# tatsuya-ogawa/GaussianSplattingMlx

Hardware: AMD Instinct MI355X
Metric: train views/sec (full step: fwd + L1/DSSIM loss + bwd + Adam + densify/prune at the reference cadence), Lego 800x800 300k Gaussians (higher is better)
Workload: dtype f32; 1 GPU; c3_300k_800: synthetic Lego cameras 800x800, N=300000 trained-like Gaussians, SH degree 4 (K=25), 16x16 tiles, 100 views, 1 view per rank per step, mode train; mode=train, parallelism=dp1, rccl_ranks=1, view_assignment=rank r renders view (step * world + r) mod views; parameters replicated, views_per_rank=1, N=300000, W=800, H=800, tile=16

## Files before the change

gaussiansplattingmlx_amd/_lib.py:

```python
from __future__ import annotations

import ctypes as C
import os

HERE = os.path.dirname(os.path.abspath(__file__))
LIB_PATH = os.environ.get("GSPLAT_LIB", os.path.join(HERE, "libgsplat_hip.so"))

GS_OK = 0
MAX_FEATURE_CHANNELS = 256
STATUS = {1: "GS_ERR_INVALID_ARG", 2: "GS_ERR_SIZE_MISMATCH", 3: "GS_ERR_WORKSPACE_OVERFLOW", 4: "GS_ERR_HIP",
          5: "GS_ERR_NO_FORWARD", 6: "GS_ERR_NO_DEVICE", 7: "GS_ERR_IO", 8: "GS_ERR_COMM", 9: "GS_ERR_REPLICA_MISMATCH"}
GS_ERR_REPLICA_MISMATCH = 9


class GsplatError(RuntimeError):
    def __init__(self, code, msg):
        super().__init__(f"{STATUS.get(code, code)}: {msg}")
        self.code = code


class gs_camera(C.Structure):
    _fields_ = [("view", C.c_float * 16), ("proj", C.c_float * 16), ("cam_center", C.c_float * 3),
                ("fov_x", C.c_float), ("fov_y", C.c_float), ("focal_x", C.c_float), ("focal_y", C.c_float)]

# ... 99 lines not shown
    "gs_ssim_forward": (C.c_int, [_vp] + [C.c_int] * 4 + [_vp] * 9),
    "gs_ssim_backward": (C.c_int, [_vp] + [C.c_int] * 4 + [_vp] * 11),
    "gs_render_forward": (C.c_int, [_vp, C.c_int, C.c_int] + [_vp] * 6 + [C.POINTER(gs_camera)] + [_vp] * 4),
    "gs_render_backward": (C.c_int, [_vp] + [_vp] * 9),
    "gs_render_backward_dp": (C.c_int, [_vp] + [_vp] * 8),
    "gs_render_backward_adam": (C.c_int, [_vp] * 7 + [C.c_longlong, _vp, C.c_float, C.c_float, C.c_float, C.c_float]),
    "gs_render_backward_dp_begin": (C.c_int, [_vp] * 5),
    "gs_render_backward_dp_finish": (C.c_int, [_vp] * 5),
    "gs_render_backward_dp_finish_geom": (C.c_int, [_vp] * 6),
    "gs_render_backward_dp_geom": (C.c_int, [_vp] * 10),
    "gs_sh_grad_from_views_adam_dir": (C.c_int, [_vp, C.c_int, C.c_int, C.c_int] + [_vp] * 9 + [C.c_longlong] + [C.c_float] * 6 + [_vp]),
    "gs_adam_step_add": (C.c_int, [_vp, C.c_longlong] + [_vp] * 4 + [C.c_int, _vp, _vp] + [C.c_float] * 4 + [_vp, C.c_longlong]),
    "gs_sh_grad_from_views": (C.c_int, [_vp, C.c_int, C.c_int, C.c_int] + [_vp] * 5),
    "gs_accum_grad_norm": (C.c_int, [_vp, C.c_int, _vp, _vp, _vp]),
    "gs_classify_gaussians": (C.c_int, [_vp, C.c_int, _vp, C.c_float, _vp, C.c_int, _vp, C.c_float, C.c_float,
                                        C.c_float, C.c_int, _vp, _vp]),
    "gs_densify_offsets": (C.c_int, [_vp, C.c_int, _vp, _vp, _vp, _vp]),
    "gs_build_densify_output_map": (C.c_int, [_vp, C.c_int, _vp, _vp, C.c_int, _vp, _vp]),
    "gs_densify_gather": (C.c_int, [_vp, C.c_int, C.c_int] + [_vp] * 15),
    "gs_densify_plan": (C.c_int, [_vp, C.c_int, _vp, _vp, _vp]),
    "gs_densify_plan_read": (C.c_int, [_vp, C.c_int, _vp, C.POINTER(C.c_int)]),
    "gs_build_densify_output_map_planned": (C.c_int, [_vp, C.c_int, _vp, _vp, C.c_int, _vp, _vp]),
    "gs_densify_gather_planned": (C.c_int, [_vp, C.c_int, C.c_int] + [_vp] * 8 + [C.c_ulonglong] + [_vp] * 6),
    "gs_densify_gather_planned_packed": (C.c_int, [_vp, C.c_int, C.c_int] + [_vp] * 8 + [C.c_ulonglong, _vp, C.POINTER(C.c_int)]),
    "gs_densify_noise": (C.c_int, [_vp, C.c_ulonglong, C.c_int, _vp]),
    "gs_ply_write": (C.c_int, [_vp, C.c_char_p, C.c_int, C.c_int] + [_vp] * 6),
    "gs_ply_probe": (C.c_int, [_vp, C.c_char_p, _vp, _vp, _vp]),
    "gs_ply_load": (C.c_int, [_vp, C.c_char_p, C.c_int, C.c_int] + [_vp] * 6),
    "gs_ply_pack_rows": (C.c_int, [_vp, C.c_int, C.c_int] + [_vp] * 7),
    "gs_set_block_work_buffer": (C.c_int, [_vp, _vp]),
    "gs_view_hint_words": (C.c_int, [_vp, C.POINTER(C.c_int)]),
    "gs_set_view_hints": (C.c_int, [_vp, _vp, C.c_int]),
    "gs_set_depth_cuts": (C.c_int, [_vp, C.c_int]),
    "gs_clear_depth_cuts": (C.c_int, [_vp, _vp, C.c_int]),
    "gs_forward_missed": (C.c_int, [_vp, C.POINTER(C.c_int)]),
    "gs_cut_stats": (C.c_int, [_vp, C.POINTER(C.c_uint32)]),
    "gs_set_grad_norm_accum": (C.c_int, [_vp, _vp]),
    "gs_block_count": (C.c_int, [_vp, _vp]),
    "gs_copy_block_work": (C.c_int, [_vp, _vp]),
    "gs_dist_topk": (C.c_int, [_vp, C.c_int, C.c_int, C.c_int, C.c_int, _vp, _vp]),
    "gs_sh_grad_from_views_adam": (C.c_int, [_vp, C.c_int, C.c_int, C.c_int] + [_vp] * 8 + [C.c_longlong] + [C.c_float] * 6),
    "gs_loss_target_cache_floats": (C.c_int, [_vp, C.POINTER(C.c_longlong)]),
    "gs_set_loss_target_cache": (C.c_int, [_vp, _vp, C.c_int]),
    "gs_set_loss_mask": (C.c_int, [_vp, _vp]),
    "gs_loss_forward_backward": (C.c_int, [_vp] + [_vp] * 5 + [C.c_float, C.c_float] + [_vp] * 3),
    "gs_depth_loss": (C.c_int, [_vp, C.POINTER(gs_depth_loss_params)] + [_vp] * 7),
    "gs_depth_normalize": (C.c_int, [_vp, C.c_longlong, _vp, _vp, C.c_float, _vp]),
    "gs_normal_loss": (C.c_int, [_vp, C.POINTER(gs_normal_loss_params)] + [_vp] * 9),
    "gs_depth_normals": (C.c_int, [_vp, C.POINTER(C.c_float), C.c_int, C.c_int, _vp, _vp, C.c_float, C.c_float, _vp]),
    "gs_image_metrics": (C.c_int, [_vp, C.c_int, C.c_int] + [_vp] * 4),
    "gs_colour_moments": (C.c_int, [_vp, C.c_longlong] + [_vp] * 4),
    "gs_adam_step": (C.c_int, [_vp, C.c_longlong] + [_vp] * 4 + [C.c_int, _vp, _vp] + [C.c_float] * 4),
    "gs_profile_enable": (C.c_int, [_vp, C.c_uint]),
    "gs_profile_read": (C.c_int, [_vp, _vp, _vp]),
    "gs_copy_last_contrib": (C.c_int, [_vp, _vp]),
    "gs_last_stats": (C.c_int, [_vp, C.POINTER(C.c_uint32)]),
    "gs_ctx_set_tuning": (C.c_int, [_vp, C.c_int, C.c_longlong]),
    "gs_copy_overflow_flag": (C.c_int, [_vp, _vp]),
    "gs_set_update_gate": (C.c_int, [_vp, _vp]),
    "gs_set_overflow_rider": (C.c_int, [_vp, _vp]),
    "gs_set_pose_correction": (C.c_int, [_vp, _vp, _vp]),
    "gs_set_exposure": (C.c_int, [_vp, _vp, _vp]),
    "gs_apply_exposure": (C.c_int, [_vp, C.c_longlong, _vp, _vp, _vp]),
    "gs_set_bilateral_grid": (C.c_int, [_vp, _vp, _vp, C.c_int, C.c_int, C.c_int, C.c_float]),
    "gs_apply_bilateral_grid": (C.c_int, [_vp, C.c_int, C.c_int, _vp, C.c_int, C.c_int, C.c_int, _vp, _vp]),
    "gs_set_antialiasing": (C.c_int, [_vp, C.c_int]),
    "gs_set_camera_model": (C.c_int, [_vp, C.c_int]),
    "gs_get_camera_model": (C.c_int, [_vp, C.POINTER(C.c_int)]),
    "gs_set_sh_degree": (C.c_int, [_vp, C.c_int]),
    "gs_get_sh_degree": (C.c_int, [_vp, C.POINTER(C.c_int)]),
    "gs_set_background": (C.c_int, [_vp, _vp]),
    "gs_get_background": (C.c_int, [_vp, _vp]),
    "gs_composite_target": (C.c_int, [_vp, C.c_longlong, _vp, _vp, _vp, _vp]),
    "gs_set_absgrad": (C.c_int, [_vp, C.c_int]),
    "gs_get_absgrad": (C.c_int, [_vp, C.c_int, _vp]),
    "gs_set_adc_stats": (C.c_int, [_vp, _vp, _vp, _vp]),
    "gs_adc_accumulate": (C.c_int, [_vp, C.c_int, _vp, _vp, C.c_int, _vp, _vp, _vp]),
    "gs_adc_classify": (C.c_int, [_vp, C.c_int] + [_vp] * 4 + [C.c_int, _vp, C.POINTER(gs_adc_params), C.c_int, C.c_int, _vp, _vp]),
    "gs_adc_gather": (C.c_int, [_vp, C.c_int, C.c_int] + [_vp] * 9 + [C.c_int] + [_vp] * 6),
    "gs_adc_gather_moments": (C.c_int, [_vp, C.c_int, C.c_int, _vp, _vp, _vp, C.POINTER(_vp), C.POINTER(_vp)]),
    "gs_adc_reset_opacity": (C.c_int, [_vp, C.c_int, _vp, _vp, _vp, C.c_float]),
    "gs_set_sparse_adam": (C.c_int, [_vp, C.c_int]),
    "gs_get_visibility": (C.c_int, [_vp, C.c_int, _vp]),
    "gs_adam_step_visible": (C.c_int, [_vp, C.c_longlong] + [_vp] * 4 + [C.c_int, _vp, _vp, _vp] + [C.c_float] * 4 + [C.c_int, _vp]),
    "gs_set_filter3d_cameras": (C.c_int, [_vp, C.c_int, _vp]),
    "gs_compute_filter3d": (C.c_int, [_vp, C.c_int, _vp, _vp]),
    "gs_set_filter3d": (C.c_int, [_vp, _vp]),
    "gs_filter3d_bake": (C.c_int, [_vp, C.c_int] + [_vp] * 5),
    "gs_undistort": (C.c_int, [_vp, C.POINTER(gs_lens)] + [C.c_int] * 6 + [_vp, _vp, _vp]),
    "gs_undistort_fisheye": (C.c_int, [_vp, C.POINTER(gs_fisheye_lens)] + [C.c_int] * 6 + [_vp, _vp, _vp]),
    "gs_tsdf_integrate": (C.c_int, [_vp, C.POINTER(gs_tsdf_grid), C.c_int, C.POINTER(gs_tsdf_view)] + [_vp] * 4),
    "gs_tsdf_mesh_workspace_bytes": (C.c_size_t, [C.POINTER(gs_tsdf_grid)]),
    "gs_tsdf_mesh_plan": (C.c_int, [_vp, C.POINTER(gs_tsdf_grid), _vp, _vp, C.c_float, _vp, C.c_size_t, C.POINTER(C.c_longlong)]),
    "gs_tsdf_mesh_emit": (C.c_int, [_vp, C.POINTER(gs_tsdf_grid), _vp, _vp, _vp, _vp, C.c_float, _vp, _vp, _vp, _vp]),
    "gs_set_mcmc": (C.c_int, [_vp, _vp]),
    "gs_mcmc_regularizer_grad": (C.c_int, [_vp, C.c_int] + [_vp] * 5),
    "gs_mcmc_inject_noise": (C.c_int, [_vp, C.c_int] + [_vp] * 4 + [C.c_float, _vp]),
    "gs_mcmc_random": (C.c_int, [_vp, C.c_ulonglong, C.c_int, C.c_int, C.c_int, _vp, _vp, _vp]),
    "gs_mcmc_relocate": (C.c_int, [_vp, C.c_int, C.c_int] + [_vp] * 11),
    "gs_mcmc_grow": (C.c_int, [_vp, C.c_int, C.c_int, C.c_int] + [_vp] * 11),
    "gs_set_gathered_gate": (C.c_int, [_vp, C.c_longlong, C.c_int, _vp]),
    "gs_set_gate_seen": (C.c_int, [_vp, _vp]),
    "gs_dp_cc_floats": (C.c_longlong, [C.c_int]),
    "gs_dp_check_replicas": (C.c_int, [_vp, C.c_int, _vp, C.c_longlong]),
    "gs_dp_check_replicas_begin": (C.c_int, [_vp, C.c_int, _vp, C.c_longlong]),
    "gs_dp_check_replicas_end": (C.c_int, [_vp]),
    "gs_dp_check_plan": (C.c_int, [_vp, C.POINTER(C.c_longlong), C.c_int]),
}

_lib = None


def load():
    global _lib
    if _lib is not None:
        return _lib
    if not os.path.exists(LIB_PATH):
        raise ImportError(f"{LIB_PATH} is missing: run `python -m gaussiansplattingmlx_amd.build` "
                          "(or __graft_entry__.build()). There is no CPU fallback.")
    import torch
    lib = C.CDLL(LIB_PATH)
    for name, (res, args) in _SIGS.items():
        fn = getattr(lib, name)
        fn.restype = res
        fn.argtypes = args
    _lib = lib
    return lib


TUNE_FWD_WAVES_PER_SIMD, TUNE_BWD_WAVES_PER_CU, TUNE_FWD_QUADRANTS, TUNE_OP_FWD_PPL, TUNE_OP_BWD_PPL, \
    TUNE_FWD_TRACE_BUFFER, TUNE_DEPTH_GRADIENT, TUNE_WIDE_TILE_SORT, TUNE_HOST_OVERFLOW_ERRORS, TUNE_SPLITTER_DEPTH_SORT, \
    TUNE_COLOUR_RIDERS, TUNE_FWD_QUEUES, TUNE_FWD_FOUR_WAVES, TUNE_FWD_FOLD_TEST_SCALE, TUNE_POISON_CHECKPOINTS, TUNE_RENDER_ONLY, TUNE_FWD_PAIR, TUNE_FWD_SLOW_SLOT, TUNE_TRIM_RECTS, TUNE_SH_BAND_SKIP = range(20)


def exported_symbols():
    return list(_SIGS)


def make_camera(view, proj, camCenter, fovX, fovY, focalX, focalY) -> gs_camera:
    import numpy as np
    cam = gs_camera()
    v = np.asarray(view, dtype=np.float32).reshape(16)
    p = np.asarray(proj, dtype=np.float32).reshape(16)
    cc = np.asarray(camCenter, dtype=np.float32).reshape(3)
    for i in range(16):
        cam.view[i] = float(v[i])
        cam.proj[i] = float(p[i])
    for i in range(3):
        cam.cam_center[i] = float(cc[i])
    cam.fov_x, cam.fov_y, cam.focal_x, cam.focal_y = float(fovX), float(fovY), float(focalX), float(focalY)
    return cam
```

gaussiansplattingmlx_amd/build.py:

```python
from __future__ import annotations

import os
import subprocess
import sys
from concurrent.futures import ThreadPoolExecutor

HERE = os.path.dirname(os.path.abspath(__file__))
CSRC = os.path.join(HERE, "csrc")
LIB = os.path.join(HERE, "libgsplat_hip.so")
HIPCC = os.environ.get("HIPCC", "/opt/rocm/bin/hipcc")
ARCH = "gfx950"

SOURCES = {
    "api.hip": [],
    "projection.hip": ["-ffp-contract=off"],
    "binning.hip": ["-ffp-contract=off"],
    "blend.hip": [],
    "blend_v2.hip": ["-ffp-contract=off"],
    "ssim.hip": [],
    "optim.hip": [],
    "densify.hip": ["-ffp-contract=off"],
    "adc.hip": ["-ffp-contract=off"],
    "ply.hip": [],
    "knn.hip": ["-ffp-contract=off"],
    "dp.hip": [],
    "mcmc.hip": ["-ffp-contract=off"],
    "exposure.hip": ["-ffp-contract=off"],
    "bilateral_grid.hip": ["-ffp-contract=off"],
    "filter3d.hip": ["-ffp-contract=off"],
    "contrib.hip": ["-ffp-contract=off"],
    "features.hip": ["-ffp-contract=off"],
    "background.hip": ["-ffp-contract=off"],
    "depth_loss.hip": ["-ffp-contract=off"],
    "normal_loss.hip": ["-ffp-contract=off"],
    "lens.hip": ["-ffp-contract=off"],
    "metrics.hip": ["-ffp-contract=off"],
    "tsdf.hip": ["-ffp-contract=off"],
}
COMMON = ["-O3", "-std=c++17", "-fPIC", f"--offload-arch={ARCH}", "-fvisibility=hidden", "-Wall", "-fno-slp-vectorize",
          "-Wno-unused-function", "-DGSPLAT_BUILD"]


def _newer(target, deps):
    if not os.path.exists(target):
        return False
    t = os.path.getmtime(target)
    return all(os.path.getmtime(d) <= t for d in deps)


def build(force: bool = False, verbose: bool = False, variant: str = "", defines=()) -> str:
    headers = [os.path.join(CSRC, h) for h in os.listdir(CSRC) if h.endswith(".h")]
    headers.append(os.path.join(HERE, "..", "include", "gsplat.h"))
    objdir = os.path.join(HERE, "_obj" + ("_" + variant if variant else ""))
    lib = LIB if not variant else os.path.join(HERE, f"libgsplat_hip_{variant}.so")
    os.makedirs(objdir, exist_ok=True)
    jobs = []
    objs = []
    for src, extra in SOURCES.items():
        s = os.path.join(CSRC, src)
        o = os.path.join(objdir, src.replace(".hip", ".o"))
        objs.append(o)
        if force or not _newer(o, [s] + headers + [os.path.abspath(__file__)]):
            jobs.append([HIPCC, *COMMON, *extra, *defines, "-c", s, "-o", o])

    def run(cmd):
        if verbose:
            print(" ".join(cmd), flush=True)
        r = subprocess.run(cmd, capture_output=True, text=True)
        if r.returncode != 0:
            raise RuntimeError("hipcc failed:\n" + " ".join(cmd) + "\n" + r.stdout + r.stderr)
        if verbose and r.stderr.strip():
            print(r.stderr)

    if jobs:
        with ThreadPoolExecutor(max_workers=min(4, len(jobs))) as ex:
            list(ex.map(run, jobs))
    if jobs or not os.path.exists(lib):
        run([HIPCC, "-shared", "-fPIC", f"--offload-arch={ARCH}", "-o", lib, *objs, "-ldl"])
    return lib


if __name__ == "__main__":
    argv = sys.argv[1:]
    variant = argv[argv.index("--variant") + 1] if "--variant" in argv else ""
    print(build(force="--force" in argv, verbose=True, variant=variant, defines=[a for a in argv if a.startswith("-D")]))
```

gaussiansplattingmlx_amd/csrc/api.hip:

```cpp
#include <math.h>
#include <stdlib.h>
#include <stdio.h>
#include <string.h>

#include "gs_ctx.h"
#include <vector>

using namespace gs;

namespace {

int fail(gs_ctx* c, int code, const std::string& msg)
{
    if (c) c->err = msg;
    return code;
}

void free_gaussian_ws(gs_ctx* c)
{
    ctx_free(c, c->packed12); ctx_free(c, c->gradAcc16);
    for (int i = 0; i < 2; i++) { ctx_free(c, c->depthKey[i]); ctx_free(c, c->depthVal[i]); }
    ctx_free(c, c->tilesTouched); ctx_free(c, c->tileRect); ctx_free(c, c->tilePieces); ctx_free(c, c->waveSeg);
    ctx_free(c, c->scanPrefix); ctx_free(c, c->scanTmp); ctx_free(c, c->blockSums);
    ctx_free(c, c->visPerBlock); ctx_free(c, c->dropPerBlock);
// ... 385 lines not shown
    c->blocksX = gs_div_up(W, 16); c->blocksY = gs_div_up(H, 16);
    c->real.tileW = tile_w; c->real.tileH = tile_h; c->real.gridW = c->gridW; c->real.gridH = c->gridH; c->real.T = c->T;
    c->real.fast16 = c->fast16;
    {
        const char* e = getenv("GSPLAT_BLOCK_LISTS");
        const int nbx = gs_div_up(tile_w, 16), nby = gs_div_up(tile_h, 16);
        if (!c->fast16 && !(e && atoi(e) == 0) && (long long)c->gridW * nbx <= 65535 && (long long)c->gridH * nby <= 65535) {
            c->virt.nbx = nbx; c->virt.nby = nby; c->virt.tw = tile_w; c->virt.th = tile_h;
            c->tileW = 16; c->tileH = 16;
            c->gridW *= nbx; c->gridH *= nby;
            c->T = c->gridW * c->gridH;
            c->fast16 = true;
            c->blocksX = c->gridW; c->blocksY = c->gridH;
        }
    }
    if (const char* e = getenv("GSPLAT_COLOUR_RIDERS")) c->colourRiders = atoi(e);
    if (const char* e = getenv("GSPLAT_FWD_WIDE")) c->fwdWide = atoi(e) < 0 ? -1 : atoi(e) != 0;
    if (const char* e = getenv("GSPLAT_FWD_QUEUES")) { const int q = atoi(e); if (q >= 1 && q <= (int)GS_QUEUES && !(q & (q - 1))) c->fwdQueues = q; }
    if (const char* e = getenv("GSPLAT_RIDER_SHARES")) {
        int vals[GS_RIDE_HOSTS + 1], n = 0;
        for (const char* q = e; *q && n <= GS_RIDE_HOSTS; n++) {
            vals[n] = atoi(q);
            while (*q && *q != ',') q++;
            if (*q == ',') q++;
        }
        if (n == GS_RIDE_HOSTS) for (int i = 0; i < GS_RIDE_HOSTS; i++) c->riderShare[i] = vals[i];
        else fprintf(stderr, "gsplat: GSPLAT_RIDER_SHARES needs %d comma-separated values (got %s): ignored\n", GS_RIDE_HOSTS, e);
    }
    if (c->gridW > 65535 || c->gridH > 65535) { delete c; return GS_ERR_INVALID_ARG; }
    int bits = 1;
    while ((1LL << bits) < c->T) bits++;
    c->tileBits = bits;
    for (bits = 1; (1LL << bits) < c->real.T; bits++) {}
    c->real.tileBits = bits;
    auto bail = [&](int code) { gs_ctx_destroy(c); return code; };
    if (hipSetDevice(device) != hipSuccess) return bail(GS_ERR_HIP);
    if (hipStreamCreateWithFlags(&c->own_stream, hipStreamNonBlocking) != hipSuccess) return bail(GS_ERR_HIP);
    c->stream = c->own_stream;
    const size_t P = (size_t)W * H;
    c->numPixBlocks = c->blocksX * c->blocksY;
    c->opBlocks = c->real.fast16 ? c->numPixBlocks : c->real.T * gs_div_up(tile_w, 16) * gs_div_up(tile_h, 16);
    const size_t maxBlocks = (size_t)(c->opBlocks > c->numPixBlocks ? c->opBlocks : c->numPixBlocks);
    if (ctx_alloc(c, &c->blockWorkOwn, maxBlocks) || ctx_alloc(c, &c->blockOrder, maxBlocks + 8) || ctx_alloc(c, &c->fwdQueue, GS_QUEUES * GS_QUEUE_STRIDE) || ctx_alloc(c, &c->bwdQueue, GS_QUEUES * GS_QUEUE_STRIDE) ||
        ctx_alloc(c, &c->segBase, (size_t)c->numPixBlocks) || ctx_alloc(c, &c->finalT, P))
        return bail(GS_ERR_HIP);
    c->blockWork = c->blockWorkOwn;
    {
        hipDeviceProp_t prop;
        if (hipGetDeviceProperties(&prop, device) == hipSuccess && prop.multiProcessorCount > 0)
            c->numCUs = prop.multiProcessorCount;
    }
    if (ctx_alloc(c, &c->superCut, (size_t)c->T + 16) || ctx_alloc(c, &c->tileRanges, (size_t)c->T * 2) || ctx_alloc(c, &c->tileCounts, (size_t)c->T) ||
        ctx_alloc(c, &c->lastContrib, P) ||
        ctx_alloc(c, &c->lossPartials, (size_t)(c->lossPartialBlocks = gs_div_up(W, 16) * gs_div_up(H, 16) * 3) * 4 + 16) || ctx_alloc(c, &c->windowDev, 121) ||
        ctx_alloc(c, &c->counters, GS_CNT_COUNT) || ctx_alloc(c, &c->rowTotal, 256) ||
        ctx_alloc(c, &c->sortBits, GS_SMALL_SORT_BLOCKS) || ctx_alloc(c, &c->wideTotal, GS_WIDE_BINS) ||
        ctx_alloc(c, &c->bucketStart, 520) || ctx_alloc(c, &c->sortSplit[0], 256) || ctx_alloc(c, &c->sortSplit[1], 256))
        return bail(GS_ERR_HIP);
    if (ctx_alloc_pinned(c, &c->countersHost, GS_CNT_COUNT)) return bail(GS_ERR_HIP);
    if (ctx_alloc_pinned(c, &c->missHost, 16, hipHostMallocMapped)) return bail(GS_ERR_HIP);
    for (int i = 0; i < 16; i++) c->missHost[i] = 0;
    if (hipHostGetDevicePointer((void**)&c->missDev, c->missHost, 0) != hipSuccess) return bail(GS_ERR_HIP);
    if (hipEventCreateWithFlags(&c->fwdDone, hipEventDisableTiming) != hipSuccess) return bail(GS_ERR_HIP);
    float win[121];
    gs_ssim_window(11, 1.5f, win);
    if (hipMemcpy(c->windowDev, win, sizeof win, hipMemcpyHostToDevice) != hipSuccess) return bail(GS_ERR_HIP);
    if (hipMemset(c->counters, 0, sizeof(uint32_t) * GS_CNT_COUNT) != hipSuccess) return bail(GS_ERR_HIP);
    if (hipMemset(c->tileRanges, 0, sizeof(uint32_t) * 2 * c->T) != hipSuccess) return bail(GS_ERR_HIP);
    c->adamGate = c->counters + GS_CNT_OVERFLOW;
    *out = c;
    return GS_OK;
}

int gs_ctx_destroy(gs_ctx* c)
{
    if (!c) return GS_OK;
    (void)hipSetDevice(c->device);
    if (c->stream) (void)hipStreamSynchronize(c->stream);
    (void)gs_dp_shutdown(c);
    c->mem.freeAll();
    for (auto& e : c->profPool) { (void)hipEventDestroy(e.a); (void)hipEventDestroy(e.b); }
    if (c->fwdDone) (void)hipEventDestroy(c->fwdDone);
    if (c->densifyDone) (void)hipEventDestroy(c->densifyDone);
    if (c->own_stream) (void)hipStreamDestroy(c->own_stream);
    delete c;
    return GS_OK;
}

int gs_ctx_set_stream(gs_ctx* c, void* hip_stream)
{
    if (!c) return GS_ERR_INVALID_ARG;
    GS_HIP_CHECK(c, hipStreamSynchronize(c->stream));
    c->stream = (hipStream_t)hip_stream;
    return GS_OK;
}

int gs_ctx_reserve(gs_ctx* c, int max_gaussians, long long max_pairs)
{
    if (!c || max_gaussians < 0 || max_pairs < 0) return fail(c, GS_ERR_INVALID_ARG, "gs_ctx_reserve: negative size");
    (void)hipSetDevice(c->device);
    GS_HIP_CHECK(c, hipStreamSynchronize(c->stream));
    if (c->missHost[4] == 2u || c->arenaRegrowPending) {
        uint32_t parts[8], used = 0;
        GS_HIP_CHECK(c, hipMemcpy(parts, c->counters + GS_CNT_QSLOTS, sizeof parts, hipMemcpyDeviceToHost));
        for (uint32_t x : parts) used += x;
        const long long need5 = (((long long)used + c->fwd.qslotStatic) * c->fwd.statePlanes + 4) / 5;
        c->qslotWanted = need5 + need5 / 2 + 4096;
        const long long half = c->qslotCap + c->qslotCap / 2;
        if (c->qslotWanted < half) c->qslotWanted = half;
    }
    c->reserving = max_pairs > 0;
    int rc = ensure_capacity(c, max_gaussians, max_pairs);
    if (rc == GS_OK) rc = ensure_arena(c);
    c->reserving = false;
    if (rc == GS_OK) {
        if (max_pairs > 0) c->pairsReserved = true;
        c->missHost[4] = 0; c->arenaRegrowPending = false;
    }
    return rc;
}

size_t gs_workspace_bytes(const gs_ctx* c) { return c ? c->mem.deviceBytes : 0; }

int gs_sync(gs_ctx* c)
{
    if (!c) return GS_ERR_INVALID_ARG;
    const int rc = read_counters(c);
    if (rc) return rc;
    if (c->missHost[4]) {
        const uint32_t need = c->missHost[5];
        const int orc = overflow_error(c, need);
        if (c->missHost[4] == 2u) { c->arenaRegrowPending = true; c->fwd.arenaOverflow = true; }
        c->missHost[4] = 0;
        return orc;
    }
    if (c->countersHost[GS_CNT_OVERFLOW]) return overflow_error(c);
    return GS_OK;
}

int gs_overflow_pending(gs_ctx* c, uint32_t out[2])
{
    if (!c || !out) return GS_ERR_INVALID_ARG;
    out[0] = c->missHost ? c->missHost[4] : 0u;
    out[1] = c->missHost ? c->missHost[5] : 0u;
    if (out[0] == 0u && c->arenaRegrowPending) out[0] = 2u;
    return GS_OK;
}

int gs_wait(gs_ctx* c)
{
    if (!c) return GS_ERR_INVALID_ARG;
    GS_HIP_CHECK(c, hipStreamSynchronize(c->stream));
    return GS_OK;
}

const char* gs_last_error(const gs_ctx* c) { return c ? c->err.c_str() : "null context"; }

int gs_projection_forward(gs_ctx* c, int N, int K, const float* scales, const float* rotations, const float* means3d,
                          const float* shs, const gs_camera* cam, float* means2d, float* depths, float* color,
                          float* cov2d, float* conic, float* radii, float* rect_min, float* rect_max)
{
    if (!c) return GS_ERR_INVALID_ARG;
    if (N < 0 || K < 1 || !cam) return fail(c, GS_ERR_INVALID_ARG, "gs_projection_forward: bad N/K/cam");
    if ((c->modes.degree + 1) * (c->modes.degree + 1) > K) return fail(c, GS_ERR_SIZE_MISMATCH, "K smaller than (degree+1)^2");
    if (N > 0 && (!scales || !rotations || !means3d || !shs || !means2d || !depths || !color || !cov2d || !conic ||
                  !radii || !rect_min || !rect_max))
// ... 188 lines not shown

int gs_blend_features(gs_ctx* c, int N, int C, const float* packed, const float* features, float* out)
{
    if (!c) return GS_ERR_INVALID_ARG;
    if (const int prc = blend_features_preflight(c, "gs_blend_features", N, C, packed, features, out)) return prc;
    RealGeomScope real(c);
    c->fwd.valid = false; c->fwd.bwdPrepared = false;
    if (const int rc = launch_pack11_to_12(c, N, packed)) return rc;
    return launch_blend_features(c, C, features, out);
}

int gs_blend_features_backward(gs_ctx* c, int N, int C, const float* packed, const float* cot, float* grad_features)
{
    if (!c) return GS_ERR_INVALID_ARG;
    if (const int prc = blend_features_preflight(c, "gs_blend_features_backward", N, C, packed, cot, grad_features)) return prc;
    RealGeomScope real(c);
    c->fwd.valid = false; c->fwd.bwdPrepared = false;
    if (const int rc = launch_pack11_to_12(c, N, packed)) return rc;
    return launch_blend_features_backward(c, C, cot, grad_features);
}

int gs_feature_channel_group(void) { return feature_channel_group(); }

int gs_ssim_window(int K, float sigma, float* window)
{
    if (K <= 0 || K > 32 || !window) return GS_ERR_INVALID_ARG;
    float g[32];
    const float center = (float)K / 2.0f;
    float sum = 0.0f;
    for (int x = 0; x < K; x++) {
        const float d = (float)x - center;
        g[x] = expf(-(d * d) / (2.0f * (sigma * sigma)));
        sum += g[x];
    }
    for (int x = 0; x < K; x++) g[x] = g[x] / sum;
    for (int i = 0; i < K; i++)
        for (int j = 0; j < K; j++) window[i * K + j] = g[i] * g[j];
    return GS_OK;
}

int gs_ssim_forward(gs_ctx* c, int H, int W, int C, int K, const float* img1, const float* img2, const float* window,
                    float* out_ssim, float* out_mu1, float* out_mu2, float* out_sigma1, float* out_sigma2,
                    float* out_sigma12)
{
    if (!c) return GS_ERR_INVALID_ARG;
    if (H < 0 || W < 0 || C < 0 || K <= 0 || K > 32) return fail(c, GS_ERR_INVALID_ARG, "gs_ssim_forward: bad shape");
    if (C > 65535) return fail(c, GS_ERR_INVALID_ARG, "gs_ssim_forward: too many channels");
    if ((size_t)H * W * C > 0 && (!img1 || !img2 || !window || !out_ssim || !out_mu1 || !out_mu2 || !out_sigma1 ||
                                  !out_sigma2 || !out_sigma12))
        return fail(c, GS_ERR_INVALID_ARG, "gs_ssim_forward: null buffer");
    return launch_ssim_forward(c, H, W, C, K, img1, img2, window, out_ssim, out_mu1, out_mu2, out_sigma1, out_sigma2,
                               out_sigma12);
}

int gs_ssim_backward(gs_ctx* c, int H, int W, int C, int K, const float* grad_out, const float* img1,
                     const float* img2, const float* window, const float* mu1, const float* mu2, const float* sigma1,
                     const float* sigma2, const float* sigma12, float* grad_img1, float* grad_img2)
{
    if (!c) return GS_ERR_INVALID_ARG;
    if (H < 0 || W < 0 || C < 0 || K <= 0 || K > 32) return fail(c, GS_ERR_INVALID_ARG, "gs_ssim_backward: bad shape");
    if ((size_t)H * W * C > 0 && (!grad_out || !img1 || !img2 || !window || !mu1 || !mu2 || !sigma1 || !sigma2 ||
                                  !sigma12 || !grad_img1 || !grad_img2))
        return fail(c, GS_ERR_INVALID_ARG, "gs_ssim_backward: null buffer");
    return launch_ssim_backward(c, H, W, C, K, grad_out, 0.0f, img1, img2, window, mu1, mu2, sigma1, sigma2, sigma12,
                                grad_img1, grad_img2, 0.0f);
}

int gs_render_forward(gs_ctx* c, int N, int K, const float* xyz, const float* features_dc,
                      const float* features_rest, const float* scales, const float* rotation, const float* opacity,
                      const gs_camera* cam, float* out_color, float* out_depth, float* out_alpha, float* radii)
{
    if (!c) return GS_ERR_INVALID_ARG;
    if (N < 0 || K < 1 || !cam) return fail(c, GS_ERR_INVALID_ARG, "gs_render_forward: bad N/K/cam");
    if ((c->modes.degree + 1) * (c->modes.degree + 1) > K) return fail(c, GS_ERR_SIZE_MISMATCH, "K smaller than (degree+1)^2");
    if (!out_color || !out_alpha) return fail(c, GS_ERR_INVALID_ARG, "gs_render_forward: null output");
    if (N > 0 && (!xyz || !features_dc || (K > 1 && !features_rest) || !scales || !rotation || !opacity))
        return fail(c, GS_ERR_INVALID_ARG, "gs_render_forward: null parameter tensor");
    if (c->modes.fisheye && c->modes.poseDelta)
        return fail(c, GS_ERR_INVALID_ARG, "gs_render_forward: the fisheye camera model has no pose refinement (gs_set_pose_correction is set)");
    if (c->modes.fisheye && c->modes.filter3d)
        return fail(c, GS_ERR_INVALID_ARG, "gs_render_forward: the fisheye camera model has no 3-D filter (gs_set_filter3d is set)");
    c->fwd.valid = false;
    c->visN = -1;
    const bool keepRadii = c->sparseAdam || c->adcGradSum != nullptr;
    if (keepRadii && N > c->visCap) {
        if (const int arc = ctx_grow_pair(c, &c->visMask, &c->visRadii, &c->visCap, N > c->capN ? N : c->capN)) return arc;
    }
    if (keepRadii && !radii) radii = c->visRadii;
    c->binIsBlockLists = c->virt.nbx != 0;
    const bool reserved = c->pairsReserved && c->capN >= N;
    if (reserved) { const int orc = deferred_overflow(c); if (orc) return orc; }
    if (c->fwd.cutsActive && !c->fwd.missChecked) GS_HIP_CHECK(c, hipEventSynchronize(c->fwdDone));
    c->fwd.missed = false;
    c->fwd.bwdPrepared = false;
    c->fwd.arenaOverflow = false;
    c->fwd.cutStore = c->cutStore;
    c->fwd.cutsActive = c->cutStore != nullptr && c->allowCuts && N > 0;
    c->fwd.missChecked = !c->fwd.cutsActive;
    if (c->fwd.cutsActive) c->missHost[0] = 0;
    const CamParams cp = make_cam(cam, c->W, c->H);
    if (c->modes.poseDelta) {
        if (const int arc = ctx_grow(c, &c->posePartials, &c->posePartialsCap, pose_partials_floats(N))) return arc;
        if (const int prc = launch_pose_camera(c, cp, c->modes.poseDelta)) return prc;
    }
    c->segBaseWanted = c->fast16 && N > 0;
    c->segBaseDone = false;
    c->fwdPairNow = c->fast16 && blend_forward_v2_pair_decide(c);
    int rc = bin_with_capacity(c, N, reserved, !c->fast16, [&]() {
        return launch_projection_fused_forward(c, N, K, xyz, features_dc, features_rest, scales, rotation, opacity, cp,
                                               radii);
    });
    c->segBaseWanted = false;
    if (rc) { c->rider.on = false; return rc; }
    if (c->rider.on && c->rider.next < c->rider.total) {
        GsStageTimer t(c, GS_STAGE_PROJ_FWD, true);
        if ((rc = launch_colour_rest(c))) return rc;
    }
    c->rider.on = false;
    {
        GsStageTimer t(c, GS_STAGE_BLEND_FWD);
        rc = c->fast16 ? launch_blend_forward_v2(c, out_color, out_depth, out_alpha)
                       : launch_blend_forward(c, c->modes.bg, out_color, out_depth, out_alpha, c->lastContrib);
        if (rc) return rc;
    }
    if (c->fwd.cutsActive) GS_HIP_CHECK(c, hipEventRecord(c->fwdDone, c->stream));
    c->fwd.valid = true;
    c->absgradN = -1;
    c->fwd.blendBackwardDone = false;
    c->fwd.consumed = false;
    c->fwd.blockWork = c->blockWork;
    c->fwd.N = N; c->fwd.K = K;
    c->fwd.xyz = xyz; c->fwd.fdc = features_dc; c->fwd.frest = features_rest; c->fwd.scales = scales;
    c->fwd.rot = rotation; c->fwd.opacity = opacity;
    c->fwd.outColor = out_color; c->fwd.outDepth = out_depth; c->fwd.outAlpha = out_alpha;
    c->fwd.cam = cp;
    c->fwd.modes = c->modes;
    c->fwd.radii = keepRadii ? radii : nullptr;
    if (c->sparseAdam) c->visN = N;
    return GS_OK;
}

int gs_set_sparse_adam(gs_ctx* c, int enable)
{
    if (!c) return GS_ERR_INVALID_ARG;
    if (enable != 0 && enable != 1) return fail(c, GS_ERR_INVALID_ARG, "gs_set_sparse_adam: enable is 0 or 1");
    if (enable && c->mcmcOn)
        return fail(c, GS_ERR_INVALID_ARG, "gs_set_sparse_adam: the MCMC strategy is set (its noise and regularisers act on every Gaussian)");
    if (enable && c->modes.filter3d) return fail(c, GS_ERR_INVALID_ARG, "gs_set_sparse_adam: a 3-D filter is set (gs_set_filter3d)");
    c->sparseAdam = enable == 1;
    return GS_OK;
}

int gs_get_visibility(gs_ctx* c, int N, unsigned char* out)
{
    if (!c) return GS_ERR_INVALID_ARG;
    if (c->visN < 0)
        return fail(c, GS_ERR_NO_FORWARD, "gs_get_visibility: the last gs_render_forward was not made with sparse Adam on (gs_set_sparse_adam)");
    if (N != c->visN) return fail(c, GS_ERR_SIZE_MISMATCH, "gs_get_visibility: N differs from the forward's N");
    if (N > 0 && !out) return fail(c, GS_ERR_INVALID_ARG, "gs_get_visibility: null buffer");
    if (N > 0) GS_HIP_CHECK(c, hipMemcpyAsync(out, c->visMask, (size_t)N, hipMemcpyDeviceToDevice, c->stream));
    return GS_OK;
}

int gs_set_absgrad(gs_ctx* c, int enable)
{
    if (!c) return GS_ERR_INVALID_ARG;
// ... 435 lines not shown
    c->bgGrad = grad;
    c->bgW = grid_w;
    c->bgH = grid_h;
    c->bgL = grid_l;
    c->bgTv = tv_weight;
    return GS_OK;
}

int gs_apply_bilateral_grid(gs_ctx* c, int W, int H, const float* grid, int grid_w, int grid_h, int grid_l, const float* in,
                            float* out)
{
    if (!c) return GS_ERR_INVALID_ARG;
    if (W < 0 || H < 0) return fail(c, GS_ERR_INVALID_ARG, "gs_apply_bilateral_grid: negative image size");
    if (!bilateral_shape_ok(grid_w, grid_h, grid_l))
        return fail(c, GS_ERR_INVALID_ARG, "gs_apply_bilateral_grid: grid_w, grid_h in [2, 64] and grid_l in [2, 32]");
    if ((long long)W * H > 0 && (!grid || !in || !out)) return fail(c, GS_ERR_INVALID_ARG, "gs_apply_bilateral_grid: null buffer");
    return launch_bilateral_apply(c, W, H, grid, grid_w, grid_h, grid_l, in, out);
}

int gs_render_backward(gs_ctx* c, const float* cot_color, const float* cot_depth, const float* cot_alpha,
                       float* grad_xyz, float* grad_features_dc, float* grad_features_rest, float* grad_scales,
                       float* grad_rotation, float* grad_opacity)
{
    if (!c) return GS_ERR_INVALID_ARG;
    { const int prc = backward_preflight(c, "gs_render_backward", cot_depth != nullptr); if (prc) return prc; }
    const int N = c->fwd.N, K = c->fwd.K;
    if (!cot_color) return fail(c, GS_ERR_INVALID_ARG, "gs_render_backward: null cot_color");
    if (N > 0 && (!grad_xyz || !grad_features_dc || (K > 1 && !grad_features_rest) || !grad_scales || !grad_rotation ||
                  !grad_opacity))
        return fail(c, GS_ERR_INVALID_ARG, "gs_render_backward: null gradient buffer");
    if (const int rc = blend_backward_of_forward(c, cot_color, cot_depth, cot_alpha, c->absgrad, nullptr)) return rc;
    AbsgradScope noNorm(c);
    GsStageTimer t(c, GS_STAGE_PROJ_BWD);
    return launch_projection_fused_backward(c, grad_xyz, grad_features_dc, grad_features_rest, grad_scales, grad_rotation, grad_opacity);
}

int gs_render_contrib(gs_ctx* c, float* max_w, float* sum_w)
{
    if (!c) return GS_ERR_INVALID_ARG;
    { const int prc = backward_preflight(c, "gs_render_contrib", false); if (prc) return prc; }
    if (!max_w && !sum_w) return fail(c, GS_ERR_INVALID_ARG, "gs_render_contrib: null buffer (one of max_w, sum_w at least)");
    return launch_blend_contrib(c, max_w, sum_w);
}

int gs_render_features(gs_ctx* c, int C, const float* features, float* out)
{
    if (!c) return GS_ERR_INVALID_ARG;
    { const int prc = backward_preflight(c, "gs_render_features", false); if (prc) return prc; }
    if (C < 1 || C > GS_MAX_FEATURE_CHANNELS) return fail(c, GS_ERR_INVALID_ARG, "gs_render_features: C must be in [1, GS_MAX_FEATURE_CHANNELS]");
    if (!features || !out) return fail(c, GS_ERR_INVALID_ARG, "gs_render_features: null buffer");
    return launch_blend_features(c, C, features, out);
}

int gs_render_features_backward(gs_ctx* c, int C, const float* cot, float* grad_features)
{
    if (!c) return GS_ERR_INVALID_ARG;
    { const int prc = backward_preflight(c, "gs_render_features_backward", false); if (prc) return prc; }
    if (C < 1 || C > GS_MAX_FEATURE_CHANNELS) return fail(c, GS_ERR_INVALID_ARG, "gs_render_features_backward: C must be in [1, GS_MAX_FEATURE_CHANNELS]");
    if (!cot || !grad_features) return fail(c, GS_ERR_INVALID_ARG, "gs_render_features_backward: null buffer");
    return launch_blend_features_backward(c, C, cot, grad_features);
}

int gs_contrib_actions(gs_ctx* c, int N, const float* score, float threshold, int* actions, int* output_counts)
{
    if (!c) return GS_ERR_INVALID_ARG;
    if (N < 0 || !(threshold == threshold) || (N > 0 && (!score || !actions || !output_counts)))
        return fail(c, GS_ERR_INVALID_ARG, "gs_contrib_actions: bad arguments");
    return launch_contrib_actions(c, N, score, threshold, actions, output_counts);
}

int gs_render_backward_adam(gs_ctx* c, const float* cot_color, const float* cot_depth, const float* cot_alpha,
                            float* params_base, float* m_base, float* v_base, long long n_arena, const float lr[6],
                            float beta1, float beta2, float eps, float grad_scale)
{
    if (!c) return GS_ERR_INVALID_ARG;
    { const int prc = backward_preflight(c, "gs_render_backward_adam", cot_depth != nullptr); if (prc) return prc; }
    const int N = c->fwd.N, K = c->fwd.K;
    if (!cot_color || !lr || n_arena < 0 || (N > 0 && (!params_base || !m_base || !v_base)))
        return fail(c, GS_ERR_INVALID_ARG, "gs_render_backward_adam: null buffer");
    if (const int rc = forward_in_arena(c, "gs_render_backward_adam", params_base, n_arena)) return rc;
    if (c->sparseAdam && (c->visN != N || c->fwd.modes.filter3d))
        return fail(c, GS_ERR_NO_FORWARD, "gs_render_backward_adam: sparse Adam is on, but the forward was not made under it "
                                          "(gs_set_sparse_adam comes before gs_render_forward)");
    if (const int rc = blend_backward_of_forward(c, cot_color, cot_depth, cot_alpha, c->absgrad, c->adamGate)) return rc;
    c->fwd.consumed = true;
    AbsgradScope noNorm(c);
    GsStageTimer t(c, GS_STAGE_PROJ_BWD);
    return launch_projection_fused_backward_adam(c, params_base, m_base, v_base, lr, beta1, beta2, eps, grad_scale);
}

int gs_render_backward_dp_begin(gs_ctx* c, const float* cot_color, const float* cot_depth, const float* cot_alpha,
                                float* color_cot)
{
    if (!c) return GS_ERR_INVALID_ARG;
    if (const int rc = refuse_modes(c, "gs_render_backward_dp_begin", {GS_MODE_POSE, GS_MODE_FILTER3D, GS_MODE_FISHEYE, GS_MODE_SPARSE_ADAM,
                                                                   GS_MODE_ABSGRAD, GS_MODE_ADC_STATS}))
        return rc;
    { const int prc = backward_preflight(c, "gs_render_backward_dp_begin", cot_depth != nullptr); if (prc) return prc; }
    const int N = c->fwd.N;
    if (!cot_color || (N > 0 && !color_cot)) return fail(c, GS_ERR_INVALID_ARG, "gs_render_backward_dp_begin: null buffer");
    if (const int rc = blend_backward_of_forward(c, cot_color, cot_depth, cot_alpha)) return rc;
    c->fwd.blendBackwardDone = true;
    GsStageTimer t(c, GS_STAGE_PROJ_BWD);
    return launch_color_cot(c, N, color_cot);
}

int gs_render_backward_dp_finish(gs_ctx* c, float* grad_xyz, float* grad_scales, float* grad_rotation, float* grad_opacity)
{
    if (!c) return GS_ERR_INVALID_ARG;
    if (const int rc = refuse_modes(c, "gs_render_backward_dp_finish", {GS_MODE_POSE, GS_MODE_FILTER3D, GS_MODE_FISHEYE, GS_MODE_SPARSE_ADAM})) return rc;
    if (!c->fwd.valid || !c->fwd.blendBackwardDone)
        return fail(c, GS_ERR_NO_FORWARD, "gs_render_backward_dp_finish: no gs_render_backward_dp_begin on this context");
    const int N = c->fwd.N, K = c->fwd.K;
    if (N > 0 && (!grad_xyz || !grad_scales || !grad_rotation || !grad_opacity))
        return fail(c, GS_ERR_INVALID_ARG, "gs_render_backward_dp_finish: null gradient buffer");
    c->fwd.blendBackwardDone = false;
    GsStageTimer t(c, GS_STAGE_PROJ_BWD);
    return launch_projection_fused_backward(c, grad_xyz, nullptr, nullptr, grad_scales, grad_rotation, grad_opacity, true);
}

int gs_render_backward_dp_finish_geom(gs_ctx* c, float* grad_xyz, float* grad_scales, float* grad_rotation, float* grad_opacity,
                                      float* xyz_own)
{
    if (!c) return GS_ERR_INVALID_ARG;
    if (const int rc = refuse_modes(c, "gs_render_backward_dp_finish_geom", {GS_MODE_POSE, GS_MODE_FILTER3D, GS_MODE_FISHEYE, GS_MODE_SPARSE_ADAM})) return rc;
    if (!c->fwd.valid || !c->fwd.blendBackwardDone)
        return fail(c, GS_ERR_NO_FORWARD, "gs_render_backward_dp_finish_geom: no gs_render_backward_dp_begin on this context");
    const int N = c->fwd.N;
    if (N > 0 && (!grad_xyz || !grad_scales || !grad_rotation || !grad_opacity || !xyz_own))
        return fail(c, GS_ERR_INVALID_ARG, "gs_render_backward_dp_finish_geom: null buffer");
    c->fwd.blendBackwardDone = false;
    GsStageTimer t(c, GS_STAGE_PROJ_BWD);
    return launch_projection_geom_backward(c, grad_xyz, grad_scales, grad_rotation, grad_opacity, xyz_own);
}

int gs_render_backward_dp_geom(gs_ctx* c, const float* cot_color, const float* cot_depth, const float* cot_alpha, float* color_cot,
                               float* grad_xyz, float* grad_scales, float* grad_rotation, float* grad_opacity, float* xyz_own)
{
    if (!c) return GS_ERR_INVALID_ARG;
    if (const int rc = refuse_modes(c, "gs_render_backward_dp_geom", {GS_MODE_POSE, GS_MODE_FILTER3D, GS_MODE_FISHEYE, GS_MODE_SPARSE_ADAM,
                                                                  GS_MODE_ABSGRAD, GS_MODE_ADC_STATS}))
        return rc;
    { const int prc = backward_preflight(c, "gs_render_backward_dp_geom", cot_depth != nullptr); if (prc) return prc; }
    const int N = c->fwd.N;
    if (!cot_color || (N > 0 && (!color_cot || !grad_xyz || !grad_scales || !grad_rotation || !grad_opacity || !xyz_own)))
        return fail(c, GS_ERR_INVALID_ARG, "gs_render_backward_dp_geom: null buffer");
    if (const int rc = blend_backward_of_forward(c, cot_color, cot_depth, cot_alpha)) return rc;
    GsStageTimer t(c, GS_STAGE_PROJ_BWD);
    return launch_projection_geom_backward(c, grad_xyz, grad_scales, grad_rotation, grad_opacity, xyz_own, color_cot);
}

int gs_sh_grad_from_views_adam_dir(gs_ctx* c, int N, int K, int R, const float* xyz, const float* color_cot_all,
                                   const float* cam_centers, const float* const* own_xyz, float* features_dc, float* features_rest,
                                   float* params_base, float* m_base, float* v_base, long long n_arena, float lr_dc, float lr_rest,
                                   float beta1, float beta2, float eps, float grad_scale, float* xyz_add)
{
    if (!c) return GS_ERR_INVALID_ARG;
    const char* who = "gs_sh_grad_from_views_adam_dir";
    if (const int rc = refuse_modes(c, who, {GS_MODE_SPARSE_ADAM})) return rc;
    if (const int rc = sh_views_args(c, who, N, K, R, xyz, color_cot_all, cam_centers, features_dc, features_rest, n_arena < 0,
                                     !params_base || !m_base || !v_base || !xyz_add))
        return rc;
    if ((uintptr_t)xyz_add & 15) return fail(c, GS_ERR_INVALID_ARG, "gs_sh_grad_from_views_adam_dir: xyz_add must be 16-byte aligned");
    if (const int rc = sh_in_arena(c, who, N, K, features_dc, features_rest, params_base, n_arena)) return rc;
    if (const int rc = sh_rest_alignment(c, who, N, K, features_rest, params_base, m_base, v_base)) return rc;
    if (const int rc = sh_views_gate_layout(c, who, N, R)) return rc;
    GsStageTimer t(c, GS_STAGE_ADAM);
    return launch_sh_views_dir_adam(c, N, K, R, xyz, color_cot_all, cam_centers, own_xyz, features_dc, features_rest, params_base,
                                    m_base, v_base, lr_dc, lr_rest, beta1, beta2, eps, grad_scale, xyz_add);
}

// ... 236 lines not shown
    GS_HIP_CHECK(c, hipMemsetAsync(buf + c->numPixBlocks, 0, sizeof(uint32_t) * (size_t)c->T, c->stream));
    return GS_OK;
}

int gs_set_depth_cuts(gs_ctx* c, int enable)
{
    if (!c) return GS_ERR_INVALID_ARG;
    c->allowCuts = enable != 0;
    return GS_OK;
}

int gs_forward_missed(gs_ctx* c, int* missed)
{
    if (!c || !missed) return GS_ERR_INVALID_ARG;
    *missed = 0;
    if (!c->fwd.valid) return fail(c, GS_ERR_NO_FORWARD, "gs_forward_missed: no gs_render_forward on this context");
    { const int orc = deferred_overflow(c); if (orc) return orc; }
    if (!c->fwd.cutsActive) return GS_OK;
    const int rc = settle_cut_forward(c);
    if (rc) return rc;
    *missed = c->fwd.missed ? 1 : 0;
    return deferred_overflow(c);
}

int gs_cut_stats(gs_ctx* c, uint32_t out[2])
{
    if (!c || !out) return GS_ERR_INVALID_ARG;
    out[0] = out[1] = 0;
    if (!c->fwd.valid || !c->fwd.cutsActive) return GS_OK;
    if (!c->fwd.missChecked) return fail(c, GS_ERR_INVALID_ARG, "gs_cut_stats: ask gs_forward_missed first");
    out[0] = c->missHost[1]; out[1] = c->missHost[2];
    return GS_OK;
}

int gs_ctx_set_tuning(gs_ctx* c, int knob, long long value)
{
    if (!c) return GS_ERR_INVALID_ARG;
    switch (knob) {
    case GS_TUNE_FWD_WAVES_PER_SIMD:
        if (value < 1 || value > 16) return fail(c, GS_ERR_INVALID_ARG, "gs_ctx_set_tuning: forward waves per SIMD must be 1..16");
        c->fwdWavesPerSimd = (int)value; return GS_OK;
    case GS_TUNE_BWD_WAVES_PER_CU:
        if (value < 1 || value > 64) return fail(c, GS_ERR_INVALID_ARG, "gs_ctx_set_tuning: backward waves per CU must be 1..64");
        c->bwdWavesPerCu = (int)value; return GS_OK;
    case GS_TUNE_FWD_QUADRANTS:
        c->fwdQuadrants = value != 0; return GS_OK;
    case GS_TUNE_FWD_QUEUES:
        if (value < 1 || value > (long long)GS_QUEUES || (value & (value - 1))) return fail(c, GS_ERR_INVALID_ARG, "gs_ctx_set_tuning: forward queues must be 1, 2, 4 or 8");
        c->fwdQueues = (int)value; return GS_OK;
    case GS_TUNE_FWD_FOUR_WAVES:
        c->fwdWide = value < 0 ? -1 : (value != 0); return GS_OK;
    case GS_TUNE_OP_FWD_PPL:
    case GS_TUNE_OP_BWD_PPL:
        if (value != 1 && value != 2 && value != 4) return fail(c, GS_ERR_INVALID_ARG, "gs_ctx_set_tuning: pixels per lane must be 1, 2 or 4");
        (knob == GS_TUNE_OP_FWD_PPL ? c->opFwdPpl : c->opBwdPpl) = (int)value; return GS_OK;
    case GS_TUNE_WIDE_TILE_SORT:
        c->wideTileSort = value != 0; return GS_OK;
    case GS_TUNE_DEPTH_GRADIENT:
        c->depthGradient = value != 0; return GS_OK;
    case GS_TUNE_HOST_OVERFLOW_ERRORS:
        c->hostOverflowErrors = value != 0; return GS_OK;
    case GS_TUNE_SPLITTER_DEPTH_SORT:
        c->splitterSort = value > 0; c->haveSplitters = false; return GS_OK;
    case GS_TUNE_COLOUR_RIDERS:
        c->colourRiders = (int)value; return GS_OK;
    case GS_TUNE_FWD_FOLD_TEST_SCALE:
        if (value < 1 || value > 1000) return fail(c, GS_ERR_INVALID_ARG, "gs_ctx_set_tuning: fold test scale is in permille, 1..1000");
        c->fwdFoldScale = (float)value / 1000.0f; return GS_OK;
    case GS_TUNE_POISON_CHECKPOINTS:
        c->poisonCheckpoints = value != 0; return GS_OK;
    case GS_TUNE_RENDER_ONLY:
        c->renderOnly = value != 0; return GS_OK;
    case GS_TUNE_FWD_SLOW_SLOT:
        if (value < 1 || value > 16) return fail(c, GS_ERR_INVALID_ARG, "gs_ctx_set_tuning: the first slow wave slot must be 1..16 (16 = none)");
        c->fwdSlowSlot = (int)value; return GS_OK;
    case GS_TUNE_FWD_PAIR:
        if (value < -1 || value > 16) return fail(c, GS_ERR_INVALID_ARG, "gs_ctx_set_tuning: forward pair workgroups per CU must be -1 (by list depth), 0..16");
        c->fwdPair = (int)value; return GS_OK;
    case GS_TUNE_TRIM_RECTS:
        if (value < 0 || value > 2) return fail(c, GS_ERR_INVALID_ARG, "gs_ctx_set_tuning: trim rects is 0 (the reference's squares), 1 (cut by the ellipse's box) or 2 (and into four row groups)");
        c->trimRects = value != 0; c->rowGroups = value == 2; return GS_OK;
    case GS_TUNE_SH_BAND_SKIP:
        c->shBandSkip = value != 0; return GS_OK;
    case GS_TUNE_FWD_TRACE_BUFFER:
        c->fwdTrace = reinterpret_cast<unsigned long long*>((uintptr_t)value); return GS_OK;
    default:
        return fail(c, GS_ERR_INVALID_ARG, "gs_ctx_set_tuning: unknown knob");
    }
}

int gs_copy_overflow_flag(gs_ctx* c, uint32_t* out)
{
    if (!c || !out) return GS_ERR_INVALID_ARG;
    hipLaunchKernelGGL(copy_word_kernel, dim3(1), dim3(1), 0, c->stream, c->counters + GS_CNT_OVERFLOW, out);
    GS_HIP_CHECK(c, hipGetLastError());
    return GS_OK;
}

int gs_set_update_gate(gs_ctx* c, const uint32_t* gate)
{
    if (!c) return GS_ERR_INVALID_ARG;
    c->adamGate = gate ? gate : c->counters + GS_CNT_OVERFLOW;
    return GS_OK;
}

int gs_set_overflow_rider(gs_ctx* c, float* dst)
{
    if (!c) return GS_ERR_INVALID_ARG;
    c->overflowRider = dst;
    return GS_OK;
}

int gs_set_gathered_gate(gs_ctx* c, long long block_floats, int count, uint32_t* reduced_out)
{
    if (!c) return GS_ERR_INVALID_ARG;
    if (block_floats < 0 || (block_floats > 0 && (count < 1 || count > 16)))
        return fail(c, GS_ERR_INVALID_ARG, "gs_set_gathered_gate: bad block size / count (1..16 blocks)");
    c->ccBlockFloats = block_floats;
    c->ccBlockCount = block_floats > 0 ? count : 0;
    c->gatheredGateOut = block_floats > 0 ? reduced_out : nullptr;
    return GS_OK;
}

int gs_set_gate_seen(gs_ctx* c, uint32_t* seen)
{
    if (!c) return GS_ERR_INVALID_ARG;
    c->gateSeen = seen;
    return GS_OK;
}

int gs_set_grad_norm_accum(gs_ctx* c, float* accum)
{
    if (!c) return GS_ERR_INVALID_ARG;
    c->gradNormAccum = accum;
    return GS_OK;
}

int gs_block_count(gs_ctx* c, int* n)
{
    if (!c || !n) return GS_ERR_INVALID_ARG;
    *n = c->numPixBlocks;
    return GS_OK;
}

int gs_copy_block_work(gs_ctx* c, uint32_t* out)
{
    if (!c || !out) return GS_ERR_INVALID_ARG;
    if (!c->fwd.valid) return fail(c, GS_ERR_NO_FORWARD, "gs_copy_block_work: no gs_render_forward on this context");
    if (!c->fast16) return fail(c, GS_ERR_INVALID_ARG, "gs_copy_block_work: only for tile sizes served by the fused kernels");
    GS_HIP_CHECK(c, hipMemcpyAsync(out, c->fwd.blockWork, sizeof(uint32_t) * (size_t)c->numPixBlocks, hipMemcpyDeviceToDevice,
                                   c->stream));
    return GS_OK;
}

int gs_copy_last_contrib(gs_ctx* c, uint32_t* out)
{
    if (!c || !out) return GS_ERR_INVALID_ARG;
    if (!c->fwd.valid) return fail(c, GS_ERR_NO_FORWARD, "gs_copy_last_contrib: no gs_render_forward on this context");
    GS_HIP_CHECK(c, hipMemcpyAsync(out, c->lastContrib, sizeof(uint32_t) * (size_t)c->W * c->H, hipMemcpyDeviceToDevice,
                                   c->stream));
    return GS_OK;
}

int gs_adam_step(gs_ctx* c, long long n, float* params, const float* grads, float* m, float* v, int nseg,
                 const long long* seg_end, const float* seg_lr, float beta1, float beta2, float eps, float grad_scale)
{
// ... 283 lines not shown
```

gaussiansplattingmlx_amd/csrc/gs_ctx.h:

```cpp
#pragma once
#include <hip/hip_runtime.h>
#include <stdint.h>
#include <stdio.h>

#include <initializer_list>
#include <string>
#include <vector>

#include "../../include/gsplat.h"
#include "gs_math.h"
#include "gs_mem.h"

enum {
    GS_CNT_M = 0,
    GS_CNT_OVERFLOW = 1,
    GS_CNT_MREQ = 2,
    GS_CNT_B = 3,
    GS_CNT_NVIS = 4,
    GS_CNT_CONTRIB_LO = 5,
    GS_CNT_CONTRIB_HI = 6,
    GS_CNT_ITEMS = 9,
    GS_CNT_CUT_DROPPED = 12,
    GS_CNT_QSLOTS = 16,
    GS_CNT_COUNT = 24
// ... 108 lines not shown
    bool binIsBlockLists = false;
    int blocksX = 0, blocksY = 0;
    std::string err;

    int capN = 0;
    long long capM = 0;
    bool pairsReserved = false;
    bool reserving = false;
    GsMem mem;

    float* packed12 = nullptr;
    float* gradAcc16 = nullptr;
    uint32_t* depthKey[2] = {nullptr, nullptr};
    uint32_t* depthVal[2] = {nullptr, nullptr};
    uint32_t* tilesTouched = nullptr;
    uint4* tilePieces = nullptr;
    bool piecesValid = false;
    ushort4* tileRect = nullptr;
    uint32_t* blockSums = nullptr;
    uint32_t* visPerBlock = nullptr;
    int visBlocks = 0;
    uint32_t* pairKey[2] = {nullptr, nullptr};
    uint32_t* pairVal[2] = {nullptr, nullptr};
    uint32_t* hist = nullptr;
    uint32_t* rowTotal = nullptr;
    uint16_t* wideCnt = nullptr;
    uint32_t* wideChunk = nullptr;
    uint32_t* wideTotal = nullptr;
    uint2* sortBits = nullptr;
    uint32_t* sortSplit[2] = {nullptr, nullptr};
    int splitCur = 0;
    bool haveSplitters = false;
    unsigned char* bucketId = nullptr;
    uint32_t* bucketStart = nullptr;
    int colourRiders = 1;
    GsRiderState rider;
    int riderShare[GS_RIDE_HOSTS] = {200, 500, 300};
    int splitterSort = 1;
    int nbCap = 0;
    bool superCutReady = false;
    uint32_t* dropPerBlock = nullptr;
    int dropBlocks = 0;
    uint32_t* superCut = nullptr;
    uint32_t* tileRanges = nullptr;
    uint32_t* tileCounts = nullptr;
    uint32_t* blockWork = nullptr;
    uint32_t* blockWorkOwn = nullptr;
    uint32_t* blockOrder = nullptr;
    uint32_t* fwdQueue = nullptr;
    uint32_t* bwdQueue = nullptr;
    uint32_t* cutStore = nullptr;
    bool allowCuts = true;
    const uint32_t* opCuts = nullptr;
    unsigned long long* scanTmp = nullptr;
    unsigned long long* scanPrefix = nullptr;
    uint2* waveSeg = nullptr;
    uint32_t* missHost = nullptr;
    uint32_t* missDev = nullptr;
    hipEvent_t fwdDone = nullptr;
    const uint32_t* workHint = nullptr;
    gs::CamParams* poseCam = nullptr;
    float* posePartials = nullptr;
    long long posePartialsCap = 0;
    const float* expoM = nullptr;
    float* expoGrad = nullptr;
    float* correctedImage = nullptr;
    double* expoPartials = nullptr;
    const float* bgGrid = nullptr;
    float* bgGrad = nullptr;
    int bgW = 0, bgH = 0, bgL = 0;
    float bgTv = 0.0f;
    int bgChunks = 0, bgChunksW = 0, bgChunksH = 0;
    float* bgPartials = nullptr;
    long long bgPartialsCap = 0;
    int maxDegree = 0;
    int shBandSkip = 1;
    bool absgrad = false;
    int absgradN = -1;
    bool sparseAdam = false;
    unsigned char* visMask = nullptr;
    float* visRadii = nullptr;
    int visCap = 0;
    int visN = -1;
    float* adcGradSum = nullptr;
    float* adcCount = nullptr;
    float* adcMaxRadius = nullptr;
    float* f3dCams = nullptr;
    int f3dCamCount = 0, f3dCamCap = 0;
    uint32_t* f3dMax = nullptr;
    bool mcmcOn = false;
    gs_mcmc_params mcmc = {};
    char* mcmcWs = nullptr;
    size_t mcmcWsBytes = 0;
    long long* mcmcHost = nullptr;
    float* gradNormAccum = nullptr;
    uint32_t* segBase = nullptr;
    float* segState = nullptr;
    uint32_t* segSlot = nullptr;
    long long segCap = 0;
    long long qslotCap = 0;
    long long qslotWanted = 0;
    bool arenaRegrowPending = false;
    uint32_t* itemBlock = nullptr;
    uint32_t* itemRow = nullptr;
    long long itemCap = 0;
    float* finalT = nullptr;
    int numCUs = 256;
    int numPixBlocks = 0;
    int opBlocks = 0;
    int fwdWavesPerSimd = 4, bwdWavesPerCu = 16;
    int fwdQuadrants = 1;
    int fwdWide = -1;
    float fwdFoldScale = 1.0f;
    int fwdSlowSlot = 3;
    int fwdPair = -1;
    bool fwdPairNow = false;
    bool trimRects = true;
    bool rowGroups = true;
    int renderOnly = 0;
    int poisonCheckpoints = 0;
    int fwdQueues = 8;
    int opFwdPpl = 1, opBwdPpl = 1;
    bool segBaseWanted = false;
    bool segBaseDone = false;
    int wideTileSort = 1;
    int hostOverflowErrors = 1;
    int depthGradient = 1;
    unsigned long long* fwdTrace = nullptr;
    const uint32_t* adamGate = nullptr;
    float* overflowRider = nullptr;
    long long ccBlockFloats = 0;
    int ccBlockCount = 0;
    uint32_t* gatheredGateOut = nullptr;
    uint32_t* gateSeen = nullptr;
    uint32_t* lastContrib = nullptr;
    float* lossPartials = nullptr;
    float* lossTargetCache = nullptr;
    bool lossTargetCacheFilled = false;
    const unsigned char* lossMask = nullptr;
    int lossPartialBlocks = 0;
    double* depthLossWs = nullptr;
    float* normalWs = nullptr;
    long long normalWsFloats = 0;
    double* normalPartials = nullptr;
    double* metricsWs = nullptr;
    long long metricsWsDoubles = 0;
    float* windowDev = nullptr;
    int* densifyTiles = nullptr;
    long long densifyInts = 0;
    uint32_t* densifyPlan = nullptr;
    uint32_t* densifyPlanHost = nullptr;
    uint32_t* densifyPlanHostDev = nullptr;
    hipEvent_t densifyDone = nullptr;
    bool densifyPlanned = false;
    float** densifyTable = nullptr;
    struct {
        const void* ws = nullptr;
        gs_tsdf_grid grid = {};
        float minWeight = 0.0f;
        long long V = 0, F = 0;
    } tsdfPlan;
    uint32_t* counters = nullptr;
    uint32_t* countersHost = nullptr;

    const uint32_t* sortedIdx = nullptr;
    const uint32_t* sortedRaw = nullptr;
// ... 62 lines not shown
    const int e = c->mem.alloc((void**)p, count * sizeof(T), true, flags);
    return e ? ctx_mem_error(c, "hipHostMalloc((void**)p, count * sizeof(T), flags)", e) : GS_OK;
}
template <class T>
void ctx_free(gs_ctx* c, T*& p)
{
    if (!c->mem.free((void*)p)) {
        c->err = "ctx_free: a pointer the context does not own";
        fprintf(stderr, "gsplat: %s (%p)\n", c->err.c_str(), (void*)p);
        return;
    }
    p = nullptr;
}
template <class T, class Cap>
int ctx_grow(gs_ctx* c, T** p, Cap* cap, long long want, size_t per = 1)
{
    const char* expr = "hipMalloc((void**)p, count * sizeof(T))";
    const int e = c->mem.grow((void**)p, cap, want, per * sizeof(T), [&] {
        const hipError_t w = hipStreamSynchronize(c->stream);
        if (w != hipSuccess) expr = "hipStreamSynchronize(c->stream)";
        return (int)w;
    });
    return e ? ctx_mem_error(c, expr, e) : GS_OK;
}
template <class A, class B, class Cap>
int ctx_grow_pair(gs_ctx* c, A** a, B** b, Cap* cap, long long want)
{
    Cap capB = *cap;
    int rc = ctx_grow(c, a, cap, want);
    if (rc == GS_OK) rc = ctx_grow(c, b, &capB, want);
    if (rc) { ctx_free(c, *a); ctx_free(c, *b); *cap = 0; }
    return rc;
}

static inline int gs_div_up(long long a, long long b) { return (int)((a + b - 1) / b); }
static inline bool gs_small_depth_sort(long long n) { return gs_div_up(n, GS_SORT_THREADS * GS_SMALL_SORT_ITEMS) <= GS_SMALL_SORT_BLOCKS; }

struct GsStageTimer {
    gs_ctx* c;
    int slot = -1;
    GsStageTimer(gs_ctx* ctx, int stage, bool extra = false) : c(ctx)
    {
        if (!((c->profMask >> stage) & 1u)) return;
        if (c->profUsed == c->profPool.size()) {
            if (c->profPool.size() >= 16384) return;
            gs_ctx::ProfEvent e;
            if (hipEventCreate(&e.a) != hipSuccess) return;
            if (hipEventCreate(&e.b) != hipSuccess) { (void)hipEventDestroy(e.a); return; }
            c->profPool.push_back(e);
        }
        slot = (int)c->profUsed++;
        c->profPool[slot].stage = stage;
        c->profPool[slot].extra = extra;
        (void)hipEventRecord(c->profPool[slot].a, c->stream);
    }
    ~GsStageTimer()
    {
        if (slot >= 0) (void)hipEventRecord(c->profPool[slot].b, c->stream);
    }
};

namespace gs {

enum GsMode { GS_MODE_POSE, GS_MODE_FILTER3D, GS_MODE_FISHEYE, GS_MODE_ABSGRAD, GS_MODE_SPARSE_ADAM, GS_MODE_ADC_STATS };
int refuse_modes(gs_ctx* c, const char* who, std::initializer_list<GsMode> unserved);
int forward_in_arena(gs_ctx* c, const char* who, const float* params_base, long long n_arena);

CamParams make_cam(const gs_camera* cam, int W, int H);

int launch_projection_forward(gs_ctx* c, int N, int K, const float* scales, const float* rot, const float* means3d,
                              const float* shs, const CamParams& cam, float* means2d, float* depths, float* color,
                              float* cov2d, float* conic, float* radii, float* rectMin, float* rectMax);
int launch_projection_backward(gs_ctx* c, int N, int K, const float* scales, const float* rot, const float* means3d,
                               const float* shs, const CamParams& cam, const float* cotDepths,
                               const float* cotMeans2d, const float* cotCov2d, const float* cotColor,
                               const float* cotConic, float* gScales, float* gRot, float* gMeans, float* gShs,
                               float* gCam);
int launch_projection_fused_forward(gs_ctx* c, int N, int K, const float* xyz, const float* fdc, const float* frest,
                                    const float* scales, const float* rot, const float* opacity,
                                    const CamParams& cam, float* radii);
int launch_projection_fused_backward(gs_ctx* c, float* gXyz, float* gFdc, float* gFrest, float* gScales, float* gRot, float* gOpacity,
                                     bool emitColorCot = false);
int launch_projection_fused_backward_adam(gs_ctx* c, const float* pBase, float* mBase, float* vBase, const float lr[6], float b1,
                                          float b2, float eps, float gscale);
int launch_vis_mask(gs_ctx* c, int N, const float* radii);
bool depth_sort_takes_splitters(const gs_ctx* c, int N);
int launch_pose_camera(gs_ctx* c, const gs::CamParams& host, const float* delta);
int launch_pose_grad(gs_ctx* c, int N);
long long pose_partials_floats(int N);
int launch_exposure_apply(gs_ctx* c, long long n, const float* M, const float* in, float* out);
int launch_exposure_backward(gs_ctx* c, long long n, const float* M, const float* render, float* cot, double* partials,
                             float* grad);
long long exposure_partials_doubles();
bool bilateral_shape_ok(int gw, int gh, int gl);
int bilateral_chunks(int W, int H, int gw, int gh);
long long bilateral_partials_floats(int gw, int gh, int gl, int nch);
int launch_bilateral_apply(gs_ctx* c, int W, int H, const float* G, int gw, int gh, int gl, const float* in, float* out);
int launch_bilateral_backward(gs_ctx* c, int W, int H, const float* G, int gw, int gh, int gl, int nch, float tvWeight,
                              const float* render, float* cot, float* partials, float* grad);
int launch_composite_target(gs_ctx* c, long long n, const float* rgb, const float* alpha, const float bg[3], float* out);
long long depth_loss_ws_doubles();
int launch_depth_loss(gs_ctx* c, int mode, float lambda, float alphaMin, float scale, float offset, const float* depth,
                      const float* alpha, const float* target, const unsigned char* mask, float* loss, float* cotDepth,
                      float* cotAlpha);
int launch_depth_normalize(gs_ctx* c, long long n, const float* depth, const float* alpha, float alphaMin, float* out);
long long normal_loss_ws_floats(long long np);
long long normal_loss_ws_doubles();
int launch_depth_normals(gs_ctx* c, const gs_normal_loss_params& s, const float* depth, const float* alpha, float* out);
int launch_normal_loss(gs_ctx* c, const gs_normal_loss_params& s, const float* depth, const float* alpha, const float* target,
                       const unsigned char* mask, const float* edge, float* loss, float* normalOut, float* cotDepth,
                       float* cotAlpha, float* ws, double* partials);
long long metrics_ws_doubles(int H, int W);
int launch_image_metrics(gs_ctx* c, int H, int W, const float* render, const float* target, const unsigned char* mask, double* out);
int launch_colour_moments(gs_ctx* c, long long n, const float* render, const float* target, const unsigned char* mask, double* out);
int launch_filter3d_width(gs_ctx* c, int N, const float* xyz, float* filter);
int launch_filter3d_bake(gs_ctx* c, int N, const float* scalesRaw, const float* opacityRaw, const float* filter, float* outScales,
                         float* outOpacity);
int launch_undistort(gs_ctx* c, const gs_lens& lens, int srcW, int srcH, int dstW, int dstH, int channels, int mode, const void* src,
                     void* dst, unsigned char* valid);
int launch_undistort_fisheye(gs_ctx* c, const gs_fisheye_lens& lens, int srcW, int srcH, int dstW, int dstH, int channels, int mode, const void* src,
                     void* dst, unsigned char* valid);
int launch_colour_rest(gs_ctx* c);
int launch_color_cot(gs_ctx* c, int N, float* out);
int launch_sh_grad_from_views(gs_ctx* c, int N, int K, int R, const float* xyz, const float* mgAll,
                              const float* camCentersHost, float* gFdc, float* gFrest);
int launch_sh_grad_from_views_adam(gs_ctx* c, int N, int K, int R, const float* xyz, const float* mgAll,
                                   const float* camCentersHost, const float* fdcParam, const float* frestParam,
                                   const float* pBase, float* mBase, float* vBase, float lrDc, float lrRest, float b1,
                                   float b2, float eps, float gscale);
int launch_projection_geom_backward(gs_ctx* c, float* gXyz, float* gScales, float* gRot, float* gOpacity, float* xyzOwn,
                                    float* colorCot = nullptr);
int launch_sh_views_dir_adam(gs_ctx* c, int N, int K, int R, const float* xyz, const float* mgAll, const float* camCentersHost,
                             const float* const* ownXyzHost, const float* fdcParam, const float* frestParam, const float* pBase,
                             float* mBase, float* vBase, float lrDc, float lrRest, float b1, float b2, float eps, float gscale,
                             float* xyzAdd);
int launch_pack11_to_12(gs_ctx* c, int N, const float* packed11);
int launch_pack_gaussians(gs_ctx* c, int N, const float* means2d, const float* conic, const float* color,
                          const float* opacity, const float* depths, float* packed11);

int launch_bin_prep(gs_ctx* c, int N, const float* rectMin, const float* rectMax, const float* radii,
                    const float* depths);
int launch_binning(gs_ctx* c, int N, bool wantPlain);
int ensure_plain_sorted(gs_ctx* c);
int launch_tile_counts(gs_ctx* c);
int launch_cut_super(gs_ctx* c, const uint32_t* cuts);
int cut_super_width(const gs_ctx* c);
int launch_build_packed_tile_indices(gs_ctx* c, uint32_t B, int32_t* out);

int launch_blend_forward(gs_ctx* c, const GsBackground& bg, float* outColor, float* outDepth, float* outAlpha, uint32_t* lastContrib);
int launch_blend_backward(gs_ctx* c, const GsBackground& bg, int N, const float* cotColor, const float* cotDepth, const float* cotAlpha,
                          const float* outAlpha, const uint32_t* lastContrib);
int launch_gradacc_to_packed11(gs_ctx* c, int N, float* gradPacked11);

int launch_blend_contrib(gs_ctx* c, float* maxW, float* sumW);
int launch_contrib_actions(gs_ctx* c, int N, const float* score, float threshold, int* actions, int* outputCounts);

int launch_blend_features(gs_ctx* c, int C, const float* features, float* out);
int launch_blend_features_backward(gs_ctx* c, int C, const float* cot, float* grad);
int feature_channel_group();

int launch_blend_forward_v2(gs_ctx* c, float* outColor, float* outDepth, float* outAlpha);
int launch_blend_backward_v2(gs_ctx* c, int N, const float* cotColor, const float* cotDepth, const float* cotAlpha,
                             const float* outColor, const float* outDepth, const float* outAlpha, bool absgrad = false);
bool blend_forward_v2_pair_decide(const gs_ctx* c);

int launch_ssim_forward(gs_ctx* c, int H, int W, int C, int K, const float* img1, const float* img2,
                        const float* window, float* ssim, float* mu1, float* mu2, float* s1, float* s2, float* s12);
int launch_ssim_backward(gs_ctx* c, int H, int W, int C, int K, const float* gradOut, float gradOutConst,
// ... 76 lines not shown
```

gaussiansplattingmlx_amd/csrc/projection.hip:

```cpp
#include <type_traits>

#include "gs_ctx.h"
#include "gs_mcmc.h"
#include "gs_rider.h"

namespace gs {

constexpr int PROJ_THREADS = 256;

CamParams make_cam(const gs_camera* cam, int W, int H)
{
    CamParams p;
    for (int i = 0; i < 16; i++) { p.V[i] = cam->view[i]; p.P[i] = cam->proj[i]; }
    for (int i = 0; i < 3; i++) p.cam[i] = cam->cam_center[i];
    p.fovX = cam->fov_x; p.fovY = cam->fov_y; p.focalX = cam->focal_x; p.focalY = cam->focal_y;
    p.limX = tanf(cam->fov_x * 0.5f) * 1.3f;
    p.limY = tanf(cam->fov_y * 0.5f) * 1.3f;
    p.W = (float)W; p.H = (float)H;
    return p;
}

template <bool FISHEYE>
__device__ __forceinline__ void proj_fwd_op_body(
    int N, int K, int degree, const CamParams& cam, const float* __restrict__ scales, const float* __restrict__ rot,
    const float* __restrict__ means3d, const float* __restrict__ shs, float* __restrict__ means2d,
    float* __restrict__ depths, float* __restrict__ color, float* __restrict__ cov2d, float* __restrict__ conic,
    float* __restrict__ radii, float* __restrict__ rectMin, float* __restrict__ rectMax)
{
    const int p = blockIdx.x * PROJ_THREADS + threadIdx.x;
    if (p >= N) return;
    const float m[3] = {means3d[3 * p], means3d[3 * p + 1], means3d[3 * p + 2]};
    const float s[3] = {scales[3 * p], scales[3 * p + 1], scales[3 * p + 2]};
    const float q[4] = {rot[4 * p], rot[4 * p + 1], rot[4 * p + 2], rot[4 * p + 3]};
    ProjOut o;
    project_geometry<FISHEYE>(m, s, q, cam, o);

    const float x = m[0] - cam.cam[0], y = m[1] - cam.cam[1], z = m[2] - cam.cam[2];
    const float* sh = shs + (size_t)p * K * 3;
    float c0 = 0.f, c1 = 0.f, c2 = 0.f;
    sh_foreach(degree, x, y, z, [&](int k, float b, float, float, float) {
        if (k == 0) { c0 = b * sh[0]; c1 = b * sh[1]; c2 = b * sh[2]; }
        else { c0 += b * sh[k * 3]; c1 += b * sh[k * 3 + 1]; c2 += b * sh[k * 3 + 2]; }
    });
    c0 += 0.5f; c1 += 0.5f; c2 += 0.5f;
    color[3 * p] = c0 > 0.f ? c0 : 0.f;
    color[3 * p + 1] = c1 > 0.f ? c1 : 0.f;
    color[3 * p + 2] = c2 > 0.f ? c2 : 0.f;

    means2d[2 * p] = o.sx; means2d[2 * p + 1] = o.sy;
    depths[p] = o.depth;
#pragma unroll
    for (int k = 0; k < 4; k++) { cov2d[4 * p + k] = o.cov2d[k]; conic[4 * p + k] = o.conic[k]; }
    radii[p] = o.radius;
    rectMin[2 * p] = o.rect[0]; rectMin[2 * p + 1] = o.rect[1];
    rectMax[2 * p] = o.rect[2]; rectMax[2 * p + 1] = o.rect[3];
}

__global__ __launch_bounds__(PROJ_THREADS) void proj_fwd_op_kernel(
    int N, int K, int degree, CamParams cam, const float* __restrict__ scales, const float* __restrict__ rot,
    const float* __restrict__ means3d, const float* __restrict__ shs, float* __restrict__ means2d,
    float* __restrict__ depths, float* __restrict__ color, float* __restrict__ cov2d, float* __restrict__ conic,
    float* __restrict__ radii, float* __restrict__ rectMin, float* __restrict__ rectMax)
{
    proj_fwd_op_body<false>(N, K, degree, cam, scales, rot, means3d, shs, means2d, depths, color, cov2d, conic, radii, rectMin, rectMax);
}
__global__ __launch_bounds__(PROJ_THREADS) void proj_fwd_op_fisheye_kernel(
    int N, int K, int degree, CamParams cam, const float* __restrict__ scales, const float* __restrict__ rot,
    const float* __restrict__ means3d, const float* __restrict__ shs, float* __restrict__ means2d,
    float* __restrict__ depths, float* __restrict__ color, float* __restrict__ cov2d, float* __restrict__ conic,
    float* __restrict__ radii, float* __restrict__ rectMin, float* __restrict__ rectMax)
{
    proj_fwd_op_body<true>(N, K, degree, cam, scales, rot, means3d, shs, means2d, depths, color, cov2d, conic, radii, rectMin, rectMax);
}

template <class Load, class Store>
__device__ __forceinline__ void color_backward(int degree, int K, float x, float y, float z, const float cotCol[3],
                                               Load&& shload, Store&& shstore, float dxyz[3], float* mgOut = nullptr)
{
    float acc[3] = {0.f, 0.f, 0.f};
    sh_foreach(degree, x, y, z, [&](int k, float b, float, float, float) {
#pragma unroll
        for (int ch = 0; ch < 3; ch++) acc[ch] = (k == 0) ? b * shload(k, ch) : acc[ch] + b * shload(k, ch);
    });
    float mg[3];
// ... 1 lines not shown
    for (int ch = 0; ch < 3; ch++) mg[ch] = d_max_left(acc[ch] + 0.5f, 0.0f, cotCol[ch]);
    if (mgOut) { mgOut[0] = mg[0]; mgOut[1] = mg[1]; mgOut[2] = mg[2]; }
    float dx = 0.f, dy = 0.f, dz = 0.f;
    int written = 0;
    sh_foreach(degree, x, y, z, [&](int k, float b, float gx, float gy, float gz) {
#pragma unroll
        for (int ch = 0; ch < 3; ch++) {
            const float coef = shload(k, ch);
            shstore(k, ch, b * mg[ch]);
            const float w = coef * mg[ch];
            dx += gx * w; dy += gy * w; dz += gz * w;
        }
        written = k + 1;
    });
    for (int k = written; k < K; k++)
        for (int ch = 0; ch < 3; ch++) shstore(k, ch, 0.0f);
    dxyz[0] = dx; dxyz[1] = dy; dxyz[2] = dz;
}

template <bool FISHEYE>
__device__ __forceinline__ void proj_bwd_op_body(
    int N, int K, int degree, const CamParams& cam, const float* __restrict__ scales, const float* __restrict__ rot,
    const float* __restrict__ means3d, const float* __restrict__ shs, const float* __restrict__ cotDepths,
    const float* __restrict__ cotMeans2d, const float* __restrict__ cotCov2d, const float* __restrict__ cotColor,
    const float* __restrict__ cotConic, float* __restrict__ gScales, float* __restrict__ gRot,
    float* __restrict__ gMeans, float* __restrict__ gShs, float* __restrict__ gCam)
{
    const int p = blockIdx.x * PROJ_THREADS + threadIdx.x;
    if (p >= N) return;
    const float m[3] = {means3d[3 * p], means3d[3 * p + 1], means3d[3 * p + 2]};
    const float s[3] = {scales[3 * p], scales[3 * p + 1], scales[3 * p + 2]};
    const float q[4] = {rot[4 * p], rot[4 * p + 1], rot[4 * p + 2], rot[4 * p + 3]};
    const float cm[2] = {cotMeans2d[2 * p], cotMeans2d[2 * p + 1]};
    const float ccov[4] = {cotCov2d[4 * p], cotCov2d[4 * p + 1], cotCov2d[4 * p + 2], cotCov2d[4 * p + 3]};
    const float ccon[4] = {cotConic[4 * p], cotConic[4 * p + 1], cotConic[4 * p + 2], cotConic[4 * p + 3]};
    GeomGrads g;
    project_geometry_bwd<false, false, FISHEYE>(m, s, q, cam, cm, cotDepths[p], ccov, ccon, g);

    const float x = m[0] - cam.cam[0], y = m[1] - cam.cam[1], z = m[2] - cam.cam[2];
    const float* sh = shs + (size_t)p * K * 3;
    float* gsh = gShs + (size_t)p * K * 3;
    const float cc[3] = {cotColor[3 * p], cotColor[3 * p + 1], cotColor[3 * p + 2]};
    float d[3];
    color_backward(degree, K, x, y, z, cc, [&](int k, int ch) { return sh[k * 3 + ch]; },
                   [&](int k, int ch, float v) { gsh[k * 3 + ch] = v; }, d);
#pragma unroll
    for (int a = 0; a < 3; a++) {
        gMeans[3 * p + a] = g.dm[a] + d[a];
        gCam[3 * p + a] = -d[a];
        gScales[3 * p + a] = g.ds[a];
    }
#pragma unroll
    for (int a = 0; a < 4; a++) gRot[4 * p + a] = g.dq[a];
}

__global__ __launch_bounds__(PROJ_THREADS) void proj_bwd_op_kernel(
    int N, int K, int degree, CamParams cam, const float* __restrict__ scales, const float* __restrict__ rot,
    const float* __restrict__ means3d, const float* __restrict__ shs, const float* __restrict__ cotDepths,
    const float* __restrict__ cotMeans2d, const float* __restrict__ cotCov2d, const float* __restrict__ cotColor,
    const float* __restrict__ cotConic, float* __restrict__ gScales, float* __restrict__ gRot,
    float* __restrict__ gMeans, float* __restrict__ gShs, float* __restrict__ gCam)
{
    proj_bwd_op_body<false>(N, K, degree, cam, scales, rot, means3d, shs, cotDepths, cotMeans2d, cotCov2d, cotColor, cotConic, gScales,
                            gRot, gMeans, gShs, gCam);
}
__global__ __launch_bounds__(PROJ_THREADS) void proj_bwd_op_fisheye_kernel(
    int N, int K, int degree, CamParams cam, const float* __restrict__ scales, const float* __restrict__ rot,
    const float* __restrict__ means3d, const float* __restrict__ shs, const float* __restrict__ cotDepths,
    const float* __restrict__ cotMeans2d, const float* __restrict__ cotCov2d, const float* __restrict__ cotColor,
    const float* __restrict__ cotConic, float* __restrict__ gScales, float* __restrict__ gRot,
    float* __restrict__ gMeans, float* __restrict__ gShs, float* __restrict__ gCam)
{
    proj_bwd_op_body<true>(N, K, degree, cam, scales, rot, means3d, shs, cotDepths, cotMeans2d, cotCov2d, cotColor, cotConic, gScales,
                           gRot, gMeans, gShs, gCam);
}

constexpr int PROJ_FUSED_THREADS = 128;

constexpr int SH_ROWS_MAX4 = 18;
#ifndef GS_PROJ_LATE_MOMENTS
#define GS_PROJ_LATE_MOMENTS 1
#endif

__device__ __forceinline__ void sh_rows_load4(const float* __restrict__ g, int total4, int e0, int lane,
                                              float4 (&regs)[SH_ROWS_MAX4])
{
    const float4* g4 = reinterpret_cast<const float4*>(g);
#pragma unroll
    for (int i = 0; i < SH_ROWS_MAX4; i++) regs[i] = g4[min(e0 + lane + 64 * i, total4 - 1)];
}
__device__ __forceinline__ void sh_rows_to_lds4(float* __restrict__ lds, int total4, int L, int e0, int lane,
                                                const float4 (&regs)[SH_ROWS_MAX4])
{
#pragma unroll
    for (int i = 0; i < SH_ROWS_MAX4; i++) {
        const int e = e0 + lane + 64 * i;
        if (e < total4) {
            const int r = (e * 4) / L, c = e * 4 - r * L;
            float* d = lds + r * (L + 1) + c;
            d[0] = regs[i].x; d[1] = regs[i].y; d[2] = regs[i].z; d[3] = regs[i].w;
        }
    }
}

__device__ __forceinline__ void sh_rows_in(float* __restrict__ lds, const float* __restrict__ g, int rows, int L,
                                           int lane)
{
    const int total = rows * L;
    if ((L & 3) == 0) {
        const int total4 = total >> 2;
        for (int e0 = 0; e0 < total4; e0 += 64 * SH_ROWS_MAX4) {
            float4 regs[SH_ROWS_MAX4];
            sh_rows_load4(g, total4, e0, lane, regs);
            sh_rows_to_lds4(lds, total4, L, e0, lane, regs);
        }
    } else {
        for (int e = lane; e < total; e += 64) {
            const int r = e / L, c = e - r * L;
            lds[r * (L + 1) + c] = g[e];
        }
    }
}

__device__ __forceinline__ void sh_rows_out(const float* __restrict__ lds, float* __restrict__ g, int rows, int L,
                                            int lane)
{
    const int total = rows * L;
    if ((L & 3) == 0) {
        float4* g4 = reinterpret_cast<float4*>(g);
        for (int e = lane; e * 4 < total; e += 64) {
            const int r = (e * 4) / L, c = e * 4 - r * L;
            const float* d = lds + r * (L + 1) + c;
            g4[e] = make_float4(d[0], d[1], d[2], d[3]);
        }
    } else {
        for (int e = lane; e < total; e += 64) {
            const int r = e / L, c = e - r * L;
            g[e] = lds[r * (L + 1) + c];
        }
    }
}

#ifndef GS_DEGENERATE_INVISIBLE
#define GS_DEGENERATE_INVISIBLE 1
#endif
#include "gs_proj_fwd_kernel.h"

struct AdamFuse {
    const float* pBase;
    float* mBase;
    float* vBase;
    float lr[6];
    float b1, b2, eps, gscale;
    const uint32_t* gate;
    const uint32_t* ovf;
    float* rider;
    const uint32_t* gwWords;
    long long gwStride;
    int gwCount;
    uint32_t* gwOut;
    uint32_t* seen;
};

__device__ __forceinline__ uint32_t adam_gate_word(const AdamFuse& A)
{
    if (!A.gwWords) return A.gate ? *A.gate : 0u;
    uint32_t g = 0;
    for (int r = 0; r < A.gwCount; r++) g |= A.gwWords[(long long)r * A.gwStride];
    return g;
}
__device__ __forceinline__ void adam_gate_publish(const AdamFuse& A, uint32_t g)
{
    if (blockIdx.x == 0 && threadIdx.x == 0) {
        if (A.gwWords && A.gwOut) *A.gwOut = g;
        if (g && A.seen) *A.seen = 1u;
    }
}

__device__ __forceinline__ void adam_step(const AdamFuse& A, float g, float lr, float& p, float& m, float& v)
{
    const float gr = g * A.gscale;
    m = A.b1 * m + (1.0f - A.b1) * gr;
    v = A.b2 * v + (1.0f - A.b2) * gr * gr;
    p = p - gs_adam_delta(lr, m, v, A.eps);
}

template <bool SPARSE = false>
__device__ __forceinline__ void adam_rows(const AdamFuse& adam, const float* frest, int row0, int rows, int L,
                                          const float* myRows, int lane, float lr, unsigned long long visBits = ~0ull)
{
    const size_t off0 = (size_t)(frest - adam.pBase) + (size_t)row0 * L;
    float* P = const_cast<float*>(adam.pBase) + off0;
    float* M = adam.mBase + off0;
    float* V = adam.vBase + off0;
    const int total = rows * L;
    auto grad_at = [&](int e) { const int r = e / L; return myRows[r * (L + 1) + (e - r * L)]; };
    auto vis_at = [&](int e) { return ((visBits >> (e / L)) & 1ull) != 0ull; };
    const int head = min(total, (int)((4 - (off0 & 3)) & 3));
    const int n4 = (total - head) >> 2;
    const int tail0 = head + 4 * n4;
    if (lane < head + (total - tail0)) {
        const int e = lane < head ? lane : tail0 + (lane - head);
        bool on = true;
        if constexpr (SPARSE) on = vis_at(e);
        if (on) {
            float pv = P[e], mv = M[e], vv = V[e];
            adam_step(adam, grad_at(e), lr, pv, mv, vv);
            P[e] = pv; M[e] = mv; V[e] = vv;
        }
    }
    float4* P4 = reinterpret_cast<float4*>(P + head);
    float4* M4 = reinterpret_cast<float4*>(M + head);
    float4* V4 = reinterpret_cast<float4*>(V + head);
    if constexpr (SPARSE) {
        for (int e = lane; e < n4; e += 64) {
            const int f = head + 4 * e;
            const bool v0 = vis_at(f), v1 = vis_at(f + 1), v2 = vis_at(f + 2), v3 = vis_at(f + 3);
            if (!(v0 || v3)) continue;
            float4 p4 = P4[e], m4 = M4[e], w4 = V4[e];
            if (v0) adam_step(adam, grad_at(f), lr, p4.x, m4.x, w4.x);
            if (v1) adam_step(adam, grad_at(f + 1), lr, p4.y, m4.y, w4.y);
            if (v2) adam_step(adam, grad_at(f + 2), lr, p4.z, m4.z, w4.z);
            if (v3) adam_step(adam, grad_at(f + 3), lr, p4.w, m4.w, w4.w);
            P4[e] = p4; M4[e] = m4; V4[e] = w4;
        }
        return;
    }
    constexpr int B = 6;
    for (int e0 = lane; e0 < n4; e0 += 64 * B) {
        float4 pp[B], mm[B], vv[B];
#pragma unroll
        for (int b = 0; b < B; b++) {
            const int e = min(e0 + 64 * b, n4 - 1);
            pp[b] = P4[e]; mm[b] = M4[e]; vv[b] = V4[e];
        }
#pragma unroll
        for (int b = 0; b < B; b++) {
            const int e = e0 + 64 * b;
            if (e < n4) {
                const int f = head + 4 * e;
                adam_step(adam, grad_at(f), lr, pp[b].x, mm[b].x, vv[b].x);
                adam_step(adam, grad_at(f + 1), lr, pp[b].y, mm[b].y, vv[b].y);
                adam_step(adam, grad_at(f + 2), lr, pp[b].z, mm[b].z, vv[b].z);
                adam_step(adam, grad_at(f + 3), lr, pp[b].w, mm[b].w, vv[b].w);
                P4[e] = pp[b]; M4[e] = mm[b]; V4[e] = vv[b];
            }
        }
    }
}

template <bool SPARSE = false>
__device__ __forceinline__ void adam_rows_kept(const AdamFuse& adam, const float* frest, int row0, int total4, int L,
                                               const float* myRows, int lane, float lr,
                                               float4 (&pp)[SH_ROWS_MAX4], unsigned long long visBits = ~0ull)
{
    const size_t off0 = (size_t)(frest - adam.pBase) + (size_t)row0 * L;
    float4* P4 = reinterpret_cast<float4*>(const_cast<float*>(adam.pBase) + off0);
    float4* M4 = reinterpret_cast<float4*>(adam.mBase + off0);
    float4* V4 = reinterpret_cast<float4*>(adam.vBase + off0);
    auto grad_at = [&](int e) { const int r = e / L; return myRows[r * (L + 1) + (e - r * L)]; };
    constexpr int B = 3, NB = SH_ROWS_MAX4 / B;
    static_assert(NB * B == SH_ROWS_MAX4, "whole batches");
#ifndef GS_ADAM_ROWS_DEPTH
#define GS_ADAM_ROWS_DEPTH 2
#endif
    constexpr int D = GS_ADAM_ROWS_DEPTH;
    float4 mm[D][B], vv[D][B];
    auto vis4 = [&](int e) { return ((visBits >> ((4 * e) / L)) & 1ull) != 0ull; };
// ... 122 lines not shown
        for (int b = 0; b < B; b++) {
            const int e = min(e0 + 64 * b, total - 1), r = e / Lact, o = r * L + (e - r * Lact);
            pp[b] = P[o]; mm[b] = M[o]; vv[b] = V[o];
        }
#pragma unroll
        for (int b = 0; b < B; b++) {
            const int e = e0 + 64 * b;
            if (e < total) {
                const int r = e / Lact, c = e - r * Lact, o = r * L + c;
                adam_step(adam, myRows[r * (L + 1) + c], lr, pp[b], mm[b], vv[b]);
                P[o] = pp[b]; M[o] = mm[b]; V[o] = vv[b];
            }
        }
    }
}

__device__ __forceinline__ void drop_nonfinite_row(float4& g0, float4& g1, float4& g2)
{
#ifdef GS_KEEP_NONFINITE_ROWS
    return;
#endif
    auto fin = [](float v) { return (v - v) == 0.0f; };
    if (!(fin(g0.x) && fin(g0.y) && fin(g0.z) && fin(g0.w) && fin(g1.x) && fin(g1.y) && fin(g1.z) && fin(g1.w) && fin(g2.x) &&
          fin(g2.y) && fin(g2.z))) {
        g0 = make_float4(0.f, 0.f, 0.f, 0.f); g1 = g0; g2 = g0;
    }
}

__device__ __forceinline__ float wave_sum_xor(float v)
{
#pragma unroll
    for (int o = 32; o >= 1; o >>= 1) v += __shfl_xor(v, o, 64);
    return v;
}

template <int MODE, bool POSE, bool AA = false, bool MCMC = false, bool F3D = false, bool SPARSE = false, bool FISHEYE = false,
          bool BANDS = false>
__device__ __forceinline__ void proj_bwd_fused_body(
    int N, int K, int degree, const CamParams& cam, const float* xyz, const float* fdc,
    const float* frest, const float* scalesRaw, const float* rotRaw,
    const float* opacityRaw, const float* __restrict__ gradAcc16, float* gXyz,
    float* gFdc, float* gFrest, float* gScales, float* gRot,
    float* gOpacity, float* __restrict__ gradNormAccum, AdamFuse adam, float* __restrict__ posePartials,
    McmcFuse mc = McmcFuse{}, const float* __restrict__ filter3d = nullptr, const unsigned char* __restrict__ visMask = nullptr)
{
    constexpr bool EMIT_MG = MODE == 1, ADAM = MODE == 2;
    extern __shared__ float shLds[];
    const uint32_t gateWord = ADAM ? *adam.gate : 0u;
    const int p = blockIdx.x * PROJ_FUSED_THREADS + threadIdx.x;
    if (MODE == 0 && adam.rider && p == 0) *adam.rider = *adam.ovf ? 1.0f : 0.0f;
    const int lane = threadIdx.x & 63, wv = threadIdx.x >> 6;
    bool myVis = true;
    unsigned long long visBits = ~0ull;
    if constexpr (SPARSE) {
        myVis = p < N && visMask[p] != 0;
        visBits = __ballot(myVis);
        if (visBits == 0ull) {
            if constexpr (POSE) {
                if (lane < 16) posePartials[16 * ((size_t)blockIdx.x * (PROJ_FUSED_THREADS / 64) + wv) + lane] = 0.f;
            }
            return;
        }
    }
    const int L = (K - 1) * 3;
    float* myRows = shLds + wv * 64 * (L + 1);
    const int row0 = blockIdx.x * PROJ_FUSED_THREADS + wv * 64;
    const int rows = min(64, N - row0);
    float4 keptRows[SH_ROWS_MAX4];
    const int total4 = (rows * L) >> 2;
    bool kept = ADAM && rows > 0 && L > 0 && (L & 3) == 0 && total4 <= 64 * SH_ROWS_MAX4 &&
                (((size_t)(frest - adam.pBase) + (size_t)row0 * L) & 3) == 0;
    const int Kact = (degree + 1) * (degree + 1), Lact = 3 * (Kact - 1), A4 = (Lact + 3) >> 2, totalA = rows * A4;
    float4 bandRows[BANDS ? SH_BAND_MAX4 : 1];
    if constexpr (BANDS) {
        kept = kept && A4 <= SH_BAND_MAX4;
        if (rows > 0 && Lact > 0) {
            if (kept) {
                sh_band_load4(frest + (size_t)row0 * L, totalA, L >> 2, A4, lane, bandRows);
                sh_band_to_lds4(myRows, totalA, L, A4, lane, bandRows);
            } else sh_band_in(myRows, frest + (size_t)row0 * L, rows, L, Lact, lane);
        }
    } else
    if (kept) {
        sh_rows_load4(frest + (size_t)row0 * L, total4, 0, lane, keptRows);
        sh_rows_to_lds4(myRows, total4, L, 0, lane, keptRows);
    } else if (rows > 0 && L > 0) sh_rows_in(myRows, frest + (size_t)row0 * L, rows, L, lane);
    float pose[POSE ? 15 : 1];
    if constexpr (POSE) {
#pragma unroll
        for (int j = 0; j < 15; j++) pose[j] = 0.f;
    }
    if (p < N) {
    const float4* ga = reinterpret_cast<const float4*>(gradAcc16 + (size_t)p * 16);
    float4 g0 = ga[0], g1 = ga[1], g2 = ga[2];
    drop_nonfinite_row(g0, g1, g2);
    const float cm[2] = {g0.x, g0.y};
    const float ccon[4] = {g0.z, g0.w, g1.x, g1.y};
    const float ccol[3] = {g1.z, g1.w, g2.x};
    const float cotOpacity = g2.y, cotDepth = g2.z;
    const float ccov[4] = {0.f, 0.f, 0.f, 0.f};

    const float m[3] = {xyz[3 * p], xyz[3 * p + 1], xyz[3 * p + 2]};
    const float sr[3] = {scalesRaw[3 * p], scalesRaw[3 * p + 1], scalesRaw[3 * p + 2]};
    const float s[3] = {expf(sr[0]), expf(sr[1]), expf(sr[2])};
    const float rr[4] = {rotRaw[4 * p], rotRaw[4 * p + 1], rotRaw[4 * p + 2], rotRaw[4 * p + 3]};
    const float n2 = rr[0] * rr[0] + rr[1] * rr[1] + rr[2] * rr[2] + rr[3] * rr[3];
    const float nrm = sqrtf(n2);
    const float den = nrm + 1e-8f;
    const float q[4] = {rr[0] / den, rr[1] / den, rr[2] / den, rr[3] / den};

    GeomGrads g;
    float aaRho = 1.0f;
    const float aaSg = AA ? 1.0f / (1.0f + expf(-opacityRaw[p])) : 0.0f;
    float f3dF = 0.0f, f3dKappa = 1.0f, se[3];
    if constexpr (F3D) {
        f3dF = filter3d[p];
        f3dKappa = filter3d_activate(s, f3dF, se);
        project_geometry_bwd<POSE, AA>(m, se, q, cam, cm, cotDepth, ccov, ccon, g, POSE ? pose : nullptr, cotOpacity * aaSg * f3dKappa,
                                       &aaRho);
    } else
    project_geometry_bwd<POSE, AA, FISHEYE>(m, s, q, cam, cm, cotDepth, ccov, ccon, g, POSE ? pose : nullptr, cotOpacity * aaSg, &aaRho);
    if (g0.x == 0.f && g0.y == 0.f && g0.z == 0.f && g0.w == 0.f && g1.x == 0.f && g1.y == 0.f && g1.z == 0.f &&
        g1.w == 0.f && g2.x == 0.f && g2.y == 0.f && g2.z == 0.f) {
#pragma unroll
        for (int a = 0; a < 3; a++) { g.dm[a] = 0.f; g.ds[a] = 0.f; }
#pragma unroll
        for (int a = 0; a < 4; a++) g.dq[a] = 0.f;
        if constexpr (POSE) {
#pragma unroll
            for (int j = 0; j < 12; j++) pose[j] = 0.f;
        }
    }

    const float x = m[0] - cam.cam[0], y = m[1] - cam.cam[1], z = m[2] - cam.cam[2];
    const float* d0 = fdc + (size_t)p * 3;
    float* rest = myRows + lane * (L + 1);
    float* gd0 = gFdc + (size_t)p * 3;
    float d[3];
    const float opr = opacityRaw[p];
    float sm_[14], sv_[14], sg_[14], d0v[3] = {0.f, 0.f, 0.f};
    auto small_off = [&](int i) -> size_t {
        const float* ptr[14] = {xyz + 3 * p, xyz + 3 * p + 1, xyz + 3 * p + 2, scalesRaw + 3 * p, scalesRaw + 3 * p + 1,
                                scalesRaw + 3 * p + 2, rotRaw + 4 * p, rotRaw + 4 * p + 1, rotRaw + 4 * p + 2,
                                rotRaw + 4 * p + 3, opacityRaw + p, d0, d0 + 1, d0 + 2};
        return (size_t)(ptr[i] - adam.pBase);
    };
    if (ADAM) { d0v[0] = d0[0]; d0v[1] = d0[1]; d0v[2] = d0[2]; }
    struct __attribute__((packed, aligned(4))) V3 { float x, y, z; };
    struct __attribute__((packed, aligned(4))) V4 { float x, y, z, w; };
    auto small_moments = [&]() {
        auto in3 = [&](const float* base, int i0) {
            const size_t o = small_off(i0);
            const V3 a = *reinterpret_cast<const V3*>(adam.mBase + o), b = *reinterpret_cast<const V3*>(adam.vBase + o);
            sm_[i0] = a.x; sm_[i0 + 1] = a.y; sm_[i0 + 2] = a.z; sv_[i0] = b.x; sv_[i0 + 1] = b.y; sv_[i0 + 2] = b.z;
            (void)base;
        };
        in3(xyz, 0); in3(scalesRaw, 3); in3(fdc, 11);
        {
            const size_t o = small_off(6);
            const V4 a = *reinterpret_cast<const V4*>(adam.mBase + o), b = *reinterpret_cast<const V4*>(adam.vBase + o);
            sm_[6] = a.x; sm_[7] = a.y; sm_[8] = a.z; sm_[9] = a.w; sv_[6] = b.x; sv_[7] = b.y; sv_[8] = b.z; sv_[9] = b.w;
        }
        { const size_t o = small_off(10); sm_[10] = adam.mBase[o]; sv_[10] = adam.vBase[o]; }
    };
    if (ADAM && !GS_PROJ_LATE_MOMENTS) small_moments();
    if (EMIT_MG)
        color_backward(degree, K, x, y, z, ccol,
                       [&](int k, int ch) { return k == 0 ? d0[ch] : rest[(k - 1) * 3 + ch]; },
                       [&](int, int, float) {}, d, gFdc ? gd0 : nullptr);
    else {
        float gdc[3] = {0.f, 0.f, 0.f};
        color_backward(degree, BANDS ? Kact : K, x, y, z, ccol,
                       [&](int k, int ch) { return k == 0 ? d0[ch] : rest[(k - 1) * 3 + ch]; },
                       [&](int k, int ch, float v) {
                           if (k == 0) { if (ADAM) gdc[ch] = v; else gd0[ch] = v; }
                           else rest[(k - 1) * 3 + ch] = v;
                       }, d);
        if (ADAM) { sg_[11] = gdc[0]; sg_[12] = gdc[1]; sg_[13] = gdc[2]; }
    }
    if (ADAM && GS_PROJ_LATE_MOMENTS) small_moments();
    if constexpr (POSE) {
        const bool live = (g0.x != 0.f || g0.y != 0.f || g0.z != 0.f || g0.w != 0.f || g1.x != 0.f ||
                                                 g1.y != 0.f || g1.z != 0.f || g1.w != 0.f || g2.x != 0.f || g2.y != 0.f ||
                                                 g2.z != 0.f);
        pose[12] = live ? -d[0] : 0.f; pose[13] = live ? -d[1] : 0.f; pose[14] = live ? -d[2] : 0.f;
        bool fin = true;
#pragma unroll
        for (int j = 0; j < 15; j++) fin = fin && (pose[j] - pose[j]) == 0.0f;
        if (!fin) {
#pragma unroll
            for (int j = 0; j < 15; j++) pose[j] = 0.f;
        }
    }
    const float gx = g.dm[0] + d[0], gy = g.dm[1] + d[1], gz = g.dm[2] + d[2];
    if (ADAM) { sg_[0] = gx; sg_[1] = gy; sg_[2] = gz; }
    else { gXyz[3 * p] = gx; gXyz[3 * p + 1] = gy; gXyz[3 * p + 2] = gz; }
    if (gradNormAccum && !gateWord) gradNormAccum[p] += sqrtf(gx * gx + gy * gy + gz * gz);
    if constexpr (F3D) {
        const float sgF = 1.0f / (1.0f + expf(-opr));
        filter3d_activate<true>(s, f3dF, se, g.ds, cotOpacity * sgF * (AA ? aaRho : 1.0f) * f3dKappa);
    }
#pragma unroll
    for (int a = 0; a < 3; a++) {
        const float v = F3D ? g.ds[a] : g.ds[a] * s[a];
        if (ADAM) sg_[3 + a] = v; else gScales[3 * p + a] = v;
    }
    const float dot = g.dq[0] * rr[0] + g.dq[1] * rr[1] + g.dq[2] * rr[2] + g.dq[3] * rr[3];
    const float dn = -dot / (den * den);
    const float dn2 = dn * 0.5f / nrm;
#pragma unroll
    for (int a = 0; a < 4; a++) {
        const float v = g.dq[a] / den + 2.0f * rr[a] * dn2;
        if (ADAM) sg_[6 + a] = v; else gRot[4 * p + a] = v;
    }
    const float sg = 1.0f / (1.0f + expf(-opr));
    const float gop = (F3D ? (AA ? cotOpacity * f3dKappa * aaRho : cotOpacity * f3dKappa) : AA ? cotOpacity * aaRho : cotOpacity) * sg * (1.0f - sg);
    if (ADAM) sg_[10] = gop; else gOpacity[p] = gop;
    if constexpr (MCMC) {
        sg_[10] = sg_[10] + mc.oCoef * mcmc_sigmoid_slope(opr);
#pragma unroll
        for (int a = 0; a < 3; a++) sg_[3 + a] = sg_[3 + a] + mc.sCoef * s[a];
    }
    bool smallOn = ADAM && !gateWord;
    if constexpr (SPARSE) smallOn = smallOn && myVis;
    if (smallOn) {
        float sp[14] = {m[0], m[1], m[2], sr[0], sr[1], sr[2], rr[0], rr[1], rr[2], rr[3], opr, d0v[0], d0v[1], d0v[2]};
        const float slr[14] = {adam.lr[0], adam.lr[0], adam.lr[0], adam.lr[3], adam.lr[3], adam.lr[3], adam.lr[4],
                               adam.lr[4], adam.lr[4], adam.lr[4], adam.lr[5], adam.lr[1], adam.lr[1], adam.lr[1]};
#pragma unroll
        for (int i = 0; i < 14; i++) adam_step(adam, sg_[i], slr[i], sp[i], sm_[i], sv_[i]);
        if constexpr (MCMC) {
            float dn[3];
            mcmc_noise(mc, (uint32_t)p, sp + 3, sp + 6, sp[10], dn);
            sp[0] = sp[0] + dn[0]; sp[1] = sp[1] + dn[1]; sp[2] = sp[2] + dn[2];
        }
        float* pB = const_cast<float*>(adam.pBase);
        auto out3 = [&](int i0) {
            const size_t o = small_off(i0);
            *reinterpret_cast<V3*>(pB + o) = V3{sp[i0], sp[i0 + 1], sp[i0 + 2]};
            *reinterpret_cast<V3*>(adam.mBase + o) = V3{sm_[i0], sm_[i0 + 1], sm_[i0 + 2]};
            *reinterpret_cast<V3*>(adam.vBase + o) = V3{sv_[i0], sv_[i0 + 1], sv_[i0 + 2]};
        };
        out3(0); out3(3); out3(11);
        {
            const size_t o = small_off(6);
            *reinterpret_cast<V4*>(pB + o) = V4{sp[6], sp[7], sp[8], sp[9]};
            *reinterpret_cast<V4*>(adam.mBase + o) = V4{sm_[6], sm_[7], sm_[8], sm_[9]};
            *reinterpret_cast<V4*>(adam.vBase + o) = V4{sv_[6], sv_[7], sv_[8], sv_[9]};
        }
        { const size_t o = small_off(10); pB[o] = sp[10]; adam.mBase[o] = sm_[10]; adam.vBase[o] = sv_[10]; }
    }
    }
    if (MODE == 0 && rows > 0 && L > 0) sh_rows_out(myRows, gFrest + (size_t)row0 * L, rows, L, lane);
    if constexpr (BANDS) {
        if (!gateWord && rows > 0 && Lact > 0) {
            if (kept) adam_band_rows_kept(adam, frest, row0, totalA, L, Lact, A4, myRows, lane, adam.lr[2], bandRows);
            else adam_band_rows(adam, frest, row0, rows, L, Lact, myRows, lane, adam.lr[2]);
        }
    } else
    if (ADAM && !gateWord && rows > 0 && L > 0) {
        if (kept) adam_rows_kept<SPARSE>(adam, frest, row0, total4, L, myRows, lane, adam.lr[2], keptRows, visBits);
        else adam_rows<SPARSE>(adam, frest, row0, rows, L, myRows, lane, adam.lr[2], visBits);
    }
// ... 347 lines not shown
                                    const CamParams& cam, float* radii)
{
    if (N == 0) return GS_OK;
    const int L = (K - 1) * 3;
    const bool twoPhase = (L % 8) == 0 && L >= 48 && L / 2 <= 4 * SH_HALF_MAX4;
    const size_t lds = sizeof(float) * (PROJ_FUSED_THREADS / 64) * 64 * ((twoPhase ? L / 2 : L) + 1);
    const bool posed = c->modes.poseDelta != nullptr;
    c->rider.on = !posed && K == GS_RIDER_K && (c->colourRiders == 2 || (c->colourRiders == 1 && depth_sort_takes_splitters(c, N)));
    const bool selfColour = !posed && K == GS_RIDER_K && !c->rider.on && (c->colourRiders == 3 || c->colourRiders == 1);
    GsCutCoarse cc;
    c->dropBlocks = 0;
    if (c->fwd.cutsActive && c->fwd.cutStore && c->dropPerBlock) {
        const int src = launch_cut_super(c, c->fwd.cutStore);
        if (src) return src;
        cc.superCut = c->superCut; cc.superW = cut_super_width(c); cc.dropPerBlock = c->dropPerBlock;
        c->dropBlocks = gs_div_up(N, PROJ_FUSED_THREADS);
    }
    c->piecesValid = c->trimRects && c->rowGroups && !c->virt.nbx && c->tileW == 16 && c->tileH == 16 && c->tilePieces != nullptr;
    uint4* pieces = c->piecesValid ? c->tilePieces : nullptr;
    const int pflags = (gs_small_depth_sort(N) ? 1 : 0) | (c->trimRects ? 2 : 0);
    ColourRider a = {};
    a.xyz = xyz; a.fdc = fdc; a.frest = frest; a.packed12 = c->packed12; a.tilesTouched = c->tilesTouched;
    a.cam[0] = cam.cam[0]; a.cam[1] = cam.cam[1]; a.cam[2] = cam.cam[2];
    a.N = N; a.degree = c->modes.degree; a.unit0 = 0; a.units = gs_div_up(N, 64);
    if (c->rider.on) {
        c->rider.args = a;
        c->rider.args.units = 0;
        c->rider.next = 0;
        c->rider.total = gs_div_up(N, 64);
    }
    const bool colour = !c->rider.on && !selfColour;
    const size_t dynLds = c->rider.on ? 0 : colour ? lds : sizeof(float) * (PROJ_FUSED_THREADS / 64) * 64 * GS_RIDER_ROW;
    const int rc = with_flags(
        [&](auto TWO_PHASE, auto COLOUR, auto SELF, auto AA, auto F3D, auto POSE, auto FISHEYE) {
            if constexpr (proj_fwd_form_exists(TWO_PHASE, COLOUR, SELF, POSE, F3D, FISHEYE)) {
                hipLaunchKernelGGL((proj_fwd_fused_kernel<TWO_PHASE, COLOUR, SELF, AA, F3D, POSE, FISHEYE>), dim3(gs_div_up(N, PROJ_FUSED_THREADS)),
                                   dim3(PROJ_FUSED_THREADS), dynLds, c->stream, N, K, c->modes.degree, cam, c->tileW, c->tileH,
                                   c->gridW, c->gridH, xyz, fdc, frest, scales, rot, opacity, c->packed12, radii, c->tileRect,
                                   c->tilesTouched, c->depthKey[0], c->depthVal[0], c->visPerBlock, c->counters, pflags, a, c->virt, cc,
                                   pieces, c->modes.filter3d, c->poseCam);
                return GS_OK;
            } else {
                c->err = "fused projection forward: no kernel for this combination of settings";
                return GS_ERR_INVALID_ARG;
            }
        },
        !colour || twoPhase, colour, selfColour, c->modes.antialias, c->modes.filter3d != nullptr, posed, c->modes.fisheye);
    if (rc) return rc;
    c->visBlocks = gs_div_up(N, PROJ_FUSED_THREADS);
    GS_HIP_CHECK(c, hipGetLastError());
    if (c->sparseAdam) return launch_vis_mask(c, N, radii);
    return GS_OK;
}

int launch_vis_mask(gs_ctx* c, int N, const float* radii)
{
    if (N == 0) return GS_OK;
    if (!radii || !c->visMask || N > c->visCap) { c->err = "sparse Adam: no visibility buffers for this forward"; return GS_ERR_INVALID_ARG; }
    hipLaunchKernelGGL(vis_mask_kernel, dim3(gs_div_up(N, 256)), dim3(256), 0, c->stream, N, radii, c->visMask);
    GS_HIP_CHECK(c, hipGetLastError());
    return GS_OK;
}

__global__ __launch_bounds__(GS_RIDER_WAVES * 64) void colour_rest_kernel(ColourRider r)
{
    colour_rider_block(r, (int)blockIdx.x);
}

int launch_colour_rest(gs_ctx* c)
{
    if (!c->rider.on) return GS_OK;
    c->rider.on = false;
    const int left = c->rider.total - c->rider.next;
    if (left <= 0) return GS_OK;
    ColourRider a = c->rider.args;
    a.unit0 = c->rider.next; a.units = left;
    c->rider.next = c->rider.total;
    hipLaunchKernelGGL(colour_rest_kernel, dim3(rider_blocks(left, GS_RIDER_WAVES * 64)), dim3(GS_RIDER_WAVES * 64), 0, c->stream, a);
    GS_HIP_CHECK(c, hipGetLastError());
    return GS_OK;
}

struct ProjBwdGrads { float *xyz, *fdc, *frest, *scales, *rot, *opacity; };
static int launch_proj_bwd_fused(gs_ctx* c, int mode, const ProjBwdGrads& g, const AdamFuse& adam)
{
    const int N = c->fwd.N, K = c->fwd.K;
    if (N == 0) return c->fwd.modes.poseDelta && mode != 1 ? launch_pose_grad(c, 0) : GS_OK;
    const bool f3d = c->fwd.modes.filter3d != nullptr;
    if (f3d && mode == 1) mode = 0;
    const bool pose = c->fwd.modes.poseDelta && mode != 1;
    const bool mcmc = mode == 2 && !f3d && c->mcmcOn;
    const bool sparse = mode == 2 && !f3d && !mcmc && c->sparseAdam;
    ProjBwdArgs a = {};
    a.N = N; a.K = K; a.degree = c->fwd.modes.degree;
    a.cam = c->fwd.cam; a.dcam = c->poseCam;
    a.xyz = c->fwd.xyz; a.fdc = c->fwd.fdc; a.frest = c->fwd.frest; a.scalesRaw = c->fwd.scales; a.rotRaw = c->fwd.rot;
    a.opacityRaw = c->fwd.opacity; a.gradAcc16 = c->gradAcc16;
    a.gXyz = g.xyz; a.gFdc = g.fdc; a.gFrest = g.frest; a.gScales = g.scales; a.gRot = g.rot; a.gOpacity = g.opacity;
    a.gradNormAccum = c->gradNormAccum;
    a.adam = adam;
    a.posePartials = c->posePartials;
    if (mcmc) a.mc = mcmc_fuse(c->mcmc, N, adam.lr[0]);
    a.filter3d = c->fwd.modes.filter3d;
    a.visMask = c->visMask;
    const bool bands = mode == 2 && !pose && !mcmc && !f3d && !sparse && c->shBandSkip && (a.degree + 2) * (a.degree + 2) <= K;
    const size_t lds = bands && a.degree == 0 ? 0 : sizeof(float) * (PROJ_FUSED_THREADS / 64) * 64 * ((K - 1) * 3 + 1);
    const int rc = with_flags(
        [&](auto ADAM, auto EMIT_MG, auto POSE, auto AA, auto MCMC, auto F3D, auto SPARSE, auto FISHEYE, auto BANDS) {
            constexpr int MODE = ADAM ? 2 : EMIT_MG ? 1 : 0;
            if constexpr (!(ADAM && EMIT_MG) && proj_bwd_form_exists(MODE, POSE, MCMC, F3D, SPARSE, FISHEYE, BANDS)) {
                hipLaunchKernelGGL((proj_bwd_fused_kernel<MODE, POSE, AA, MCMC, F3D, SPARSE, FISHEYE, BANDS>), dim3(gs_div_up(N, PROJ_FUSED_THREADS)),
                                   dim3(PROJ_FUSED_THREADS), lds, c->stream, a);
                return GS_OK;
            } else {
                c->err = "fused projection backward: no kernel for this combination of settings";
                return GS_ERR_INVALID_ARG;
            }
        },
        mode == 2, mode == 1, pose, c->fwd.modes.antialias, mcmc, f3d, sparse, c->fwd.modes.fisheye, bands);
    if (rc) return rc;
    GS_HIP_CHECK(c, hipGetLastError());
    return pose ? launch_pose_grad(c, N) : GS_OK;
}

int launch_projection_fused_backward(gs_ctx* c, float* gXyz, float* gFdc, float* gFrest, float* gScales, float* gRot, float* gOpacity,
                                     bool emitColorCot)
{
    AdamFuse none = {};
    if (!emitColorCot) { none.ovf = c->counters + GS_CNT_OVERFLOW; none.rider = c->overflowRider; }
    return launch_proj_bwd_fused(c, emitColorCot ? 1 : 0, ProjBwdGrads{gXyz, gFdc, gFrest, gScales, gRot, gOpacity}, none);
}

int launch_projection_fused_backward_adam(gs_ctx* c, const float* pBase, float* mBase, float* vBase, const float lr[6], float b1,
                                          float b2, float eps, float gscale)
{
    AdamFuse a = {};
    a.pBase = pBase; a.mBase = mBase; a.vBase = vBase;
    for (int i = 0; i < 6; i++) a.lr[i] = lr[i];
    a.b1 = b1; a.b2 = b2; a.eps = eps; a.gscale = gscale;
    a.gate = c->adamGate;
    return launch_proj_bwd_fused(c, 2, ProjBwdGrads{}, a);
}

static long long cc_block_floats(const gs_ctx* c, int N) { return c->ccBlockFloats > 0 ? c->ccBlockFloats : 3LL * N; }
static void fill_gathered_gate(const gs_ctx* c, int N, const float* mgAll, AdamFuse& a)
{
    a.seen = c->gateSeen;
    if (c->ccBlockFloats <= 0) return;
    a.gwWords = reinterpret_cast<const uint32_t*>(mgAll + 3LL * N);
    a.gwStride = c->ccBlockFloats; a.gwCount = c->ccBlockCount; a.gwOut = c->gatheredGateOut;
}

int launch_color_cot(gs_ctx* c, int N, float* out)
{
    if (N == 0) return GS_OK;
    hipLaunchKernelGGL(color_cot_kernel, dim3(gs_div_up(N, 256)), dim3(256), 0, c->stream, N, c->gradAcc16, c->packed12,
                       out, c->counters + GS_CNT_OVERFLOW, c->overflowRider);
    GS_HIP_CHECK(c, hipGetLastError());
    return GS_OK;
}

int launch_sh_grad_from_views(gs_ctx* c, int N, int K, int R, const float* xyz, const float* mgAll,
                              const float* camCentersHost, float* gFdc, float* gFrest)
{
    if (N == 0) return GS_OK;
    ViewCenters v;
    v.n = R;
    for (int r = 0; r < R; r++) for (int k = 0; k < 3; k++) v.c[r][k] = camCentersHost[r * 3 + k];
    const size_t lds = sizeof(float) * (PROJ_FUSED_THREADS / 64) * 64 * ((K - 1) * 3 + 1);
    AdamFuse none = {};
    fill_gathered_gate(c, N, mgAll, none);
    hipLaunchKernelGGL(sh_grad_from_views_kernel<false>, dim3(gs_div_up(N, PROJ_FUSED_THREADS)), dim3(PROJ_FUSED_THREADS),
                       lds, c->stream, N, K, c->modes.degree, v, xyz, mgAll, cc_block_floats(c, N), gFdc, gFrest, nullptr, nullptr, none);
    GS_HIP_CHECK(c, hipGetLastError());
    return GS_OK;
}

int launch_sh_grad_from_views_adam(gs_ctx* c, int N, int K, int R, const float* xyz, const float* mgAll,
                                   const float* camCentersHost, const float* fdcParam, const float* frestParam,
                                   const float* pBase, float* mBase, float* vBase, float lrDc, float lrRest, float b1,
                                   float b2, float eps, float gscale)
{
    if (N == 0) return GS_OK;
    ViewCenters v;
    v.n = R;
    for (int r = 0; r < R; r++) for (int k = 0; k < 3; k++) v.c[r][k] = camCentersHost[r * 3 + k];
    const size_t lds = sizeof(float) * (PROJ_FUSED_THREADS / 64) * 64 * ((K - 1) * 3 + 1);
    AdamFuse a = {};
    a.pBase = pBase; a.mBase = mBase; a.vBase = vBase;
    a.lr[1] = lrDc; a.lr[2] = lrRest;
    a.b1 = b1; a.b2 = b2; a.eps = eps; a.gscale = gscale;
    a.gate = c->adamGate;
    fill_gathered_gate(c, N, mgAll, a);
    hipLaunchKernelGGL(sh_grad_from_views_kernel<true>, dim3(gs_div_up(N, PROJ_FUSED_THREADS)), dim3(PROJ_FUSED_THREADS),
                       lds, c->stream, N, K, c->modes.degree, v, xyz, mgAll, cc_block_floats(c, N), nullptr, nullptr, fdcParam, frestParam, a);
    GS_HIP_CHECK(c, hipGetLastError());
    return GS_OK;
}

int launch_projection_geom_backward(gs_ctx* c, float* gXyz, float* gScales, float* gRot, float* gOpacity, float* xyzOwn, float* colorCot)
{
    const int N = c->fwd.N;
    if (N == 0) return GS_OK;
    with_flags(
        [&](auto AA) {
            hipLaunchKernelGGL(proj_bwd_geom_kernel<AA>, dim3(gs_div_up(N, 256)), dim3(256), 0, c->stream, N, c->fwd.cam, c->fwd.xyz,
                               c->fwd.scales, c->fwd.rot, c->fwd.opacity, c->gradAcc16, gXyz, gScales, gRot, gOpacity, xyzOwn,
                               c->packed12, colorCot, c->counters + GS_CNT_OVERFLOW, c->overflowRider);
            return GS_OK;
        },
        c->fwd.modes.antialias);
    GS_HIP_CHECK(c, hipGetLastError());
    return GS_OK;
}

int launch_sh_views_dir_adam(gs_ctx* c, int N, int K, int R, const float* xyz, const float* mgAll, const float* camCentersHost,
                             const float* const* ownXyzHost, const float* fdcParam, const float* frestParam, const float* pBase,
                             float* mBase, float* vBase, float lrDc, float lrRest, float b1, float b2, float eps, float gscale,
                             float* xyzAdd)
{
    if (N == 0) return GS_OK;
    ViewCentersOwn v;
    v.n = R;
    for (int r = 0; r < 16; r++) v.own[r] = nullptr;
// ... 194 lines not shown
```

gaussiansplattingmlx_amd/renderer.py:

```python
from __future__ import annotations

import ctypes as C
import math
import os
from collections import OrderedDict, namedtuple

import numpy as np
import torch

from . import _lib, loss_mask
from ._lib import GsplatError

TILE_SIZE_H_W = namedtuple("TILE_SIZE_H_W", ["w", "h"])
RenderResult = namedtuple("RenderResult", ["render", "depth", "alpha", "visiility_filter", "radii"])


def _p(t):
    return None if t is None else C.c_void_p(t.data_ptr())


def _f32(t, device):
    if isinstance(t, torch.Tensor):
        return t.to(device=device, dtype=torch.float32).contiguous()
    return torch.as_tensor(np.ascontiguousarray(t, dtype=np.float32), device=device)
# ... 39 lines not shown
        self.device = torch.device("cuda", device)
        self.profiler = None
        torch.cuda.set_device(self.device)
        ctx = C.c_void_p()
        rc = self.lib.gs_ctx_create(device, self.W, self.H, self.TILE_SIZE.w, self.TILE_SIZE.h,
                                    self.active_sh_degree, int(self.whiteBackground), C.byref(ctx))
        if rc != _lib.GS_OK:
            raise GsplatError(rc, "gs_ctx_create failed")
        self.ctx = ctx
        self._check(self.lib.gs_ctx_set_stream(self.ctx, C.c_void_p(torch.cuda.current_stream(self.device).cuda_stream)))
        win = np.zeros(121, np.float32)
        self.lib.gs_ssim_window(11, C.c_float(1.5), win.ctypes.data_as(C.c_void_p))
        self.ssimWindow = torch.as_tensor(win, device=self.device)
        self._saved = {}
        self.reserved = None
        self._grad_norm_accum = None
        self._work_hints = {}
        self.depthCuts = True
        self._cut_policy = {}
        self._cut_view = None
        self._hinted_view = None
        self.cutMinDropped = 6_000_000
        self.cutProbeInterval = 64
        self._hints_ok = (self.TILE_SIZE.w, self.TILE_SIZE.h) == (16, 16) or \
            ((self.TILE_SIZE.w % 16 != 0 or self.TILE_SIZE.h % 16 != 0) and os.environ.get("GSPLAT_BLOCK_LISTS", "1") != "0")
        self.targetStatsCache = True
        self._target_cache = OrderedDict()
        self.targetStatsCacheBytes = 8 << 30
        self._antialiased = False
        self._camera_model = "pinhole"
        self._sh_degree = self.active_sh_degree
        self._absgrad = False
        self._sparse_adam = False
        self._background = None
        self._exposure = (None, None)
        self._bilateral = (None, None)
        self._loss_mask = None
        if antialiased:
            self.setAntialiased(True)

    def close(self):
        if getattr(self, "ctx", None):
            self.lib.gs_set_block_work_buffer(self.ctx, None)
            self.lib.gs_set_loss_target_cache(self.ctx, None, 0)
            self.lib.gs_set_loss_mask(self.ctx, None)
            self.lib.gs_set_grad_norm_accum(self.ctx, None)
            self.lib.gs_ctx_destroy(self.ctx)
            self.ctx = None

    def __del__(self):
        try:
            self.close()
        except Exception:
            pass

    def _check(self, rc):
        if rc != _lib.GS_OK:
            raise GsplatError(rc, self.lib.gs_last_error(self.ctx).decode())

    def _t(self, t):
        return _f32(t, self.device)

    def _measure(self, name, body):
        return self.profiler.measure(name, body) if self.profiler is not None else body()

    def _empty(self, *shape, dtype=torch.float32):
        return torch.empty(shape, dtype=dtype, device=self.device)

    def reserve(self, max_gaussians: int, max_pairs: int):
        self._check(self.lib.gs_ctx_reserve(self.ctx, int(max_gaussians), int(max_pairs)))
        self.reserved = (int(max_gaussians), int(max_pairs))

    def sync(self):
        self._check(self.lib.gs_sync(self.ctx))

    _TUNING = dict(fwd_waves_per_simd=_lib.TUNE_FWD_WAVES_PER_SIMD, bwd_waves_per_cu=_lib.TUNE_BWD_WAVES_PER_CU,
                   fwd_quadrants=_lib.TUNE_FWD_QUADRANTS, op_fwd_ppl=_lib.TUNE_OP_FWD_PPL,
                   op_bwd_ppl=_lib.TUNE_OP_BWD_PPL, fwd_trace_buffer=_lib.TUNE_FWD_TRACE_BUFFER,
                   depth_gradient=_lib.TUNE_DEPTH_GRADIENT, wide_tile_sort=_lib.TUNE_WIDE_TILE_SORT,
                   host_overflow_errors=_lib.TUNE_HOST_OVERFLOW_ERRORS, splitter_depth_sort=_lib.TUNE_SPLITTER_DEPTH_SORT,
                   colour_riders=_lib.TUNE_COLOUR_RIDERS, fwd_queues=_lib.TUNE_FWD_QUEUES, fwd_four_waves=_lib.TUNE_FWD_FOUR_WAVES,
                   fwd_fold_test_scale=_lib.TUNE_FWD_FOLD_TEST_SCALE, poison_checkpoints=_lib.TUNE_POISON_CHECKPOINTS,
                   render_only=_lib.TUNE_RENDER_ONLY, fwd_pair=_lib.TUNE_FWD_PAIR, fwd_slow_slot=_lib.TUNE_FWD_SLOW_SLOT,
                   trim_rects=_lib.TUNE_TRIM_RECTS, sh_band_skip=_lib.TUNE_SH_BAND_SKIP)
    _TUNING_DEFAULTS = dict(fwd_waves_per_simd=4, bwd_waves_per_cu=16, fwd_quadrants=1, op_fwd_ppl=1, op_bwd_ppl=1,
                            fwd_trace_buffer=0, depth_gradient=1, wide_tile_sort=1, host_overflow_errors=1, splitter_depth_sort=1,
                            colour_riders=1, fwd_queues=8, fwd_four_waves=-1, fwd_fold_test_scale=1000, poison_checkpoints=0, render_only=0, fwd_pair=-1, fwd_slow_slot=3, trim_rects=2,
                            sh_band_skip=1)

    def setTuning(self, **knobs):
        for k, v in knobs.items():
            self._check(self.lib.gs_ctx_set_tuning(self.ctx, self._TUNING[k], int(v)))
            self._tuning_now = {**getattr(self, "_tuning_now", {}), k: int(v)}

    def getTuning(self, knob: str) -> int:
        return getattr(self, "_tuning_now", {}).get(knob, self._TUNING_DEFAULTS[knob])

    def colourRidersActive(self, N: int, K: int = 25) -> bool:
        if K != 25 or self.getTuning("colour_riders") != 1 or ((self.TILE_SIZE.w % 16 or self.TILE_SIZE.h % 16) and not self.blockLists):
            return False
        return bool(self.getTuning("splitter_depth_sort")) and 16384 < N <= 160 * 4096

    def stats(self):
        s = (C.c_uint32 * 8)()
        self._check(self.lib.gs_last_stats(self.ctx, s))
        return dict(N_visible=s[0], M=s[1], max_tile_list=s[2], overflow=s[5], capN=s[6], capM=s[7])

    @staticmethod
    def _camera(viewMatrix, projMatrix, cameraCenter, fovX, fovY, focalX, focalY):
        g = lambda a: a.detach().cpu().numpy() if isinstance(a, torch.Tensor) else a
        return _lib.make_camera(g(viewMatrix), g(projMatrix), g(cameraCenter), float(g(fovX)), float(g(fovY)),
                                float(g(focalX)), float(g(focalY)))

    def get_scales_from(self, scales):
        return torch.exp(scales)

    def get_rotation_from(self, rotation):
        return rotation / (torch.sqrt(torch.sum(rotation * rotation, dim=1, keepdim=True)) + 1e-8)

    def get_xyz_from(self, xyz):
        return xyz

    def get_features_from(self, features_dc, features_rest):
        return torch.cat([features_dc, features_rest], dim=1)

    def get_opacity_from(self, opacity):
        return torch.sigmoid(opacity)

    def projectionScreenFused(self, scales, rotations, means3d, shs, cam):
        scales, rotations, means3d, shs = map(self._t, (scales, rotations, means3d, shs))
        N, K = means3d.shape[0], shs.shape[1]
        out = dict(means2d=self._empty(N, 2), depths=self._empty(N), color=self._empty(N, 3),
                   cov2d=self._empty(N, 2, 2), conic=self._empty(N, 2, 2), radii=self._empty(N),
                   rectMin=self._empty(N, 2), rectMax=self._empty(N, 2))
        self._check(self.lib.gs_projection_forward(
            self.ctx, N, K, _p(scales), _p(rotations), _p(means3d), _p(shs), C.byref(cam), _p(out["means2d"]),
            _p(out["depths"]), _p(out["color"]), _p(out["cov2d"]), _p(out["conic"]), _p(out["radii"]),
            _p(out["rectMin"]), _p(out["rectMax"])))
        return out

    def projectionScreenFusedVJP(self, scales, rotations, means3d, shs, cam, cotMeans2d, cotDepths, cotColor,
                                 cotCov2d, cotConic):
        scales, rotations, means3d, shs = map(self._t, (scales, rotations, means3d, shs))
        cotMeans2d, cotDepths, cotColor, cotCov2d, cotConic = map(self._t, (cotMeans2d, cotDepths, cotColor,
                                                                            cotCov2d, cotConic))
        N, K = means3d.shape[0], shs.shape[1]
        out = dict(gradScales=self._empty(N, 3), gradRot=self._empty(N, 4), gradMeans3d=self._empty(N, 3),
                   gradShs=self._empty(N, K, 3), gradCamCenterPoint=self._empty(N, 3))
        self._measure("bwd.projectionScreenFused", lambda: self._check(self.lib.gs_projection_backward(
            self.ctx, N, K, _p(scales), _p(rotations), _p(means3d), _p(shs), C.byref(cam), _p(cotDepths),
            _p(cotMeans2d), _p(cotCov2d), _p(cotColor), _p(cotConic), _p(out["gradScales"]), _p(out["gradRot"]),
            _p(out["gradMeans3d"]), _p(out["gradShs"]), _p(out["gradCamCenterPoint"]))))
        out["gradCameraCenter"] = out["gradCamCenterPoint"].sum(dim=0, keepdim=True)
        return out

    def buildGlobalTileSliceInfo(self, rect, radii, depths, want_dense: bool = False, tileCuts=None):
        rmin, rmax, radii, depths = self._t(rect[0]), self._t(rect[1]), self._t(radii), self._t(depths)
        N = radii.shape[0]
        if tileCuts is None:
            self._check(self.lib.gs_tile_bin(self.ctx, N, _p(rmin), _p(rmax), _p(radii), _p(depths)))
        else:
            cuts = torch.as_tensor(np.ascontiguousarray(tileCuts, dtype=np.uint32).view(np.int32), device=self.device)
            self._check(self.lib.gs_tile_bin_cut(self.ctx, N, _p(rmin), _p(rmax), _p(radii), _p(depths), _p(cuts)))
        M, B = C.c_uint32(), C.c_uint32()
        self._check(self.lib.gs_tile_bin_info(self.ctx, C.byref(M), C.byref(B)))
        T = ((self.W + self.TILE_SIZE.w - 1) // self.TILE_SIZE.w) * ((self.H + self.TILE_SIZE.h - 1) // self.TILE_SIZE.h)
        info = dict(M=M.value, maxTilePairs=B.value, numTiles=T)
        info["sortedGaussIdx"] = self._empty(M.value, dtype=torch.int32)
        info["tileRanges"] = self._empty(T, 2, dtype=torch.int32)
        info["tileCounts"] = self._empty(T, dtype=torch.int32)
        self._check(self.lib.gs_tile_bin_export(self.ctx, _p(info["sortedGaussIdx"]), _p(info["tileRanges"]),
# ... 1055 lines not shown
```

include/gsplat.h:

```cpp
#ifndef GSPLAT_H
#define GSPLAT_H

#include <stddef.h>
#include <stdint.h>

#ifdef __cplusplus
extern "C" {
#endif

#define GSPLAT_ABI_VERSION 6

typedef enum gs_status {
    GS_OK = 0,
    GS_ERR_INVALID_ARG = 1,
    GS_ERR_SIZE_MISMATCH = 2,
    GS_ERR_WORKSPACE_OVERFLOW = 3,
    GS_ERR_HIP = 4,
    GS_ERR_NO_FORWARD = 5,
    GS_ERR_NO_DEVICE = 6,
    GS_ERR_IO = 7,
    GS_ERR_COMM = 8,
    GS_ERR_REPLICA_MISMATCH = 9
} gs_status;

// ... 44 lines not shown
int gs_build_packed_tile_indices(gs_ctx* ctx, uint32_t B, int32_t* out);


int gs_pack_gaussians(gs_ctx* ctx, int N, const float* means2d, const float* conic, const float* color,
                      const float* opacity, const float* depths, float* packed );

int gs_blend_forward(gs_ctx* ctx, int N, const float* packed , float* out_color, float* out_depth,
                     float* out_alpha, uint32_t* last_contrib);

int gs_blend_backward(gs_ctx* ctx, int N, const float* packed, const float* cot_color, const float* cot_depth,
                      const float* cot_alpha, const float* out_color, const float* out_depth,
                      const float* out_alpha, const uint32_t* last_contrib, float* grad_packed);

int gs_blend_contrib(gs_ctx* ctx, int N, const float* packed , float* max_w ,
                     float* sum_w );

#define GS_MAX_FEATURE_CHANNELS 256
int gs_blend_features(gs_ctx* ctx, int N, int C, const float* packed , const float* features ,
                      float* out );
int gs_blend_features_backward(gs_ctx* ctx, int N, int C, const float* packed , const float* cot ,
                               float* grad_features );
int gs_feature_channel_group(void);


int gs_ssim_window(int K, float sigma, float* window );
int gs_ssim_forward(gs_ctx* ctx, int H, int W, int C, int K, const float* img1, const float* img2,
                    const float* window , float* out_ssim, float* out_mu1, float* out_mu2,
                    float* out_sigma1, float* out_sigma2, float* out_sigma12);
int gs_ssim_backward(gs_ctx* ctx, int H, int W, int C, int K, const float* grad_out, const float* img1,
                     const float* img2, const float* window, const float* mu1, const float* mu2,
                     const float* sigma1, const float* sigma2, const float* sigma12, float* grad_img1,
                     float* grad_img2);


int gs_render_forward(gs_ctx* ctx, int N, int K, const float* xyz, const float* features_dc,
                      const float* features_rest, const float* scales, const float* rotation,
                      const float* opacity, const gs_camera* cam , float* out_color, float* out_depth,
                      float* out_alpha, float* radii);

int gs_render_backward(gs_ctx* ctx, const float* cot_color, const float* cot_depth, const float* cot_alpha,
                       float* grad_xyz, float* grad_features_dc, float* grad_features_rest, float* grad_scales,
                       float* grad_rotation, float* grad_opacity);

int gs_render_backward_adam(gs_ctx* ctx, const float* cot_color, const float* cot_depth, const float* cot_alpha,
                            float* params_base, float* m_base, float* v_base, long long n_arena, const float lr[6],
                            float beta1, float beta2, float eps, float grad_scale);

int gs_render_contrib(gs_ctx* ctx, float* max_w , float* sum_w );

int gs_render_features(gs_ctx* ctx, int C, const float* features , float* out );
int gs_render_features_backward(gs_ctx* ctx, int C, const float* cot ,
                                float* grad_features );

int gs_set_pose_correction(gs_ctx* ctx, const float* delta , float* grad_delta );

int gs_set_exposure(gs_ctx* ctx, const float* M , float* grad );
int gs_apply_exposure(gs_ctx* ctx, long long n_pixels, const float* M , const float* in, float* out);

int gs_set_bilateral_grid(gs_ctx* ctx, const float* grid , float* grad , int grid_w,
                          int grid_h, int grid_l, float tv_weight);
int gs_apply_bilateral_grid(gs_ctx* ctx, int W, int H, const float* grid , int grid_w, int grid_h, int grid_l,
                            const float* in , float* out );

int gs_set_antialiasing(gs_ctx* ctx, int enable);

#define GS_CAMERA_PINHOLE 0
#define GS_CAMERA_FISHEYE 1
int gs_set_camera_model(gs_ctx* ctx, int model);
int gs_get_camera_model(gs_ctx* ctx, int* model );

int gs_set_sh_degree(gs_ctx* ctx, int degree);
int gs_get_sh_degree(gs_ctx* ctx, int* degree );

int gs_set_background(gs_ctx* ctx, const float* rgb );
int gs_get_background(gs_ctx* ctx, float rgb[3] );
int gs_composite_target(gs_ctx* ctx, long long n_pixels, const float* rgb , const float* alpha ,
                        const float* bg , float* out );

int gs_set_absgrad(gs_ctx* ctx, int enable);
int gs_get_absgrad(gs_ctx* ctx, int N, float* out );

int gs_set_sparse_adam(gs_ctx* ctx, int enable);
int gs_get_visibility(gs_ctx* ctx, int N, unsigned char* out );

int gs_set_filter3d_cameras(gs_ctx* ctx, int V, const gs_camera* cams );
int gs_compute_filter3d(gs_ctx* ctx, int N, const float* xyz , float* filter );
int gs_set_filter3d(gs_ctx* ctx, const float* filter );
int gs_filter3d_bake(gs_ctx* ctx, int N, const float* scales_raw , const float* opacity_raw ,
                     const float* filter , float* out_scales_raw , float* out_opacity_raw );

typedef struct gs_lens { float fx, fy, cx, cy, k1, k2, p1, p2; float dst_fx, dst_fy, dst_cx, dst_cy; } gs_lens;
int gs_undistort(gs_ctx* ctx, const gs_lens* lens , int src_w, int src_h, int dst_w, int dst_h, int channels,
                 int mode, const void* src , void* dst , unsigned char* valid );

typedef struct gs_fisheye_lens { float fx, fy, cx, cy, k1, k2, k3, k4; float dst_fx, dst_fy, dst_cx, dst_cy; } gs_fisheye_lens;
int gs_undistort_fisheye(gs_ctx* ctx, const gs_fisheye_lens* lens , int src_w, int src_h, int dst_w, int dst_h, int channels,
                         int mode, const void* src , void* dst , unsigned char* valid );

#define GS_TSDF_MAX_VIEWS 8
typedef struct gs_tsdf_grid { float origin[3]; float voxel; int nx, ny, nz; float trunc; } gs_tsdf_grid;
typedef struct gs_tsdf_view {
    float Rt[12];
    float fx, fy, cx, cy;
    int width, height;
    const float* depth;
    const float* color;
} gs_tsdf_view;
int gs_tsdf_integrate(gs_ctx* ctx, const gs_tsdf_grid* grid , int n_views, const gs_tsdf_view* views ,
                      float* tsdf , float* weight , float* rgb , float* cweight );
size_t gs_tsdf_mesh_workspace_bytes(const gs_tsdf_grid* grid );
int gs_tsdf_mesh_plan(gs_ctx* ctx, const gs_tsdf_grid* grid , const float* tsdf, const float* weight, float min_weight,
                      void* workspace, size_t workspace_bytes, long long* counts );
int gs_tsdf_mesh_emit(gs_ctx* ctx, const gs_tsdf_grid* grid , const float* tsdf, const float* weight, const float* rgb,
                      const float* cweight, float min_weight, void* workspace, float* vertices , float* colors ,
                      int32_t* faces );

typedef struct gs_mcmc_params {
    double noise_lr;
    double opacity_reg;
    double scale_reg;
    double min_opacity;
    double grow_rate;
    long long cap_max;
    int n_max;
    int iteration;
    unsigned long long seed;
} gs_mcmc_params;

int gs_set_mcmc(gs_ctx* ctx, const gs_mcmc_params* params );
int gs_mcmc_regularizer_grad(gs_ctx* ctx, int N, const float* scales, const float* opacity, float* grad_scales,
                             float* grad_opacity, const gs_mcmc_params* params );
int gs_mcmc_inject_noise(gs_ctx* ctx, int N, float* xyz, const float* scales, const float* rotation, const float* opacity,
                         float lr_xyz, const gs_mcmc_params* params );
int gs_mcmc_random(gs_ctx* ctx, unsigned long long seed, int iteration, int stream, int n, uint32_t* words,
                   float* normals, double* uniforms);
int gs_mcmc_relocate(gs_ctx* ctx, int N, int K, float* xyz, float* features_dc, float* features_rest, float* scales,
                     float* rotation, float* opacity, const float* param_base, float* exp_avg, float* exp_avg_sq,
                     const gs_mcmc_params* params , long long stats[4] );
int gs_mcmc_grow(gs_ctx* ctx, int N, int capacity, int K, float* xyz, float* features_dc, float* features_rest,
                 float* scales, float* rotation, float* opacity, const float* param_base, float* exp_avg, float* exp_avg_sq,
                 const gs_mcmc_params* params , int* N_out );

int gs_render_backward_dp(gs_ctx* ctx, const float* cot_color, const float* cot_depth, const float* cot_alpha,
                          float* grad_xyz, float* grad_scales, float* grad_rotation, float* grad_opacity,
                          float* color_cot );
int gs_render_backward_dp_begin(gs_ctx* ctx, const float* cot_color, const float* cot_depth, const float* cot_alpha,
                                float* color_cot );
int gs_render_backward_dp_finish(gs_ctx* ctx, float* grad_xyz, float* grad_scales, float* grad_rotation,
                                 float* grad_opacity);
int gs_sh_grad_from_views(gs_ctx* ctx, int N, int K, int R, const float* xyz, const float* color_cot_all,
                          const float* cam_centers , float* grad_features_dc, float* grad_features_rest);

int gs_sh_grad_from_views_adam(gs_ctx* ctx, int N, int K, int R, const float* xyz, const float* color_cot_all,
                               const float* cam_centers , float* features_dc, float* features_rest,
                               float* params_base, float* m_base, float* v_base, long long n_arena, float lr_dc,
                               float lr_rest, float beta1, float beta2, float eps, float grad_scale);

int gs_render_backward_dp_finish_geom(gs_ctx* ctx, float* grad_xyz, float* grad_scales, float* grad_rotation,
                                      float* grad_opacity, float* xyz_own );
int gs_render_backward_dp_geom(gs_ctx* ctx, const float* cot_color, const float* cot_depth, const float* cot_alpha,
                               float* color_cot , float* grad_xyz, float* grad_scales, float* grad_rotation,
                               float* grad_opacity, float* xyz_own );
int gs_sh_grad_from_views_adam_dir(gs_ctx* ctx, int N, int K, int R, const float* xyz, const float* color_cot_all,
                                   const float* cam_centers , const float* const* own_xyz ,
                                   float* features_dc, float* features_rest, float* params_base, float* m_base, float* v_base,
                                   long long n_arena, float lr_dc, float lr_rest, float beta1, float beta2, float eps,
// ... 130 lines not shown
int gs_adc_accumulate(gs_ctx* ctx, int N, const float* rows16, const float* radii, int use_abs, float* grad_sum, float* count,
                      float* max_radius);

typedef struct gs_adc_params {
    float grad_threshold;
    float percent_dense;
    float min_opacity;
    float max_screen_size;
    float prune_world;
    float scene_extent;
} gs_adc_params;

int gs_adc_classify(gs_ctx* ctx, int N, const float* grad_sum, const float* count, const float* max_radius,
                    const float* scales, int scale_stride, const float* opacity, const gs_adc_params* params ,
                    int allow_densify, int size_prune, int* actions, int* output_counts);
int gs_adc_gather(gs_ctx* ctx, int total, int K, const float* xyz, const float* features_dc, const float* features_rest,
                  const float* scales, const float* rotation, const float* opacity, const int* gather_indices,
                  const int* noise_mode, const float* noise, int revised_opacity, float* out_xyz, float* out_features_dc,
                  float* out_features_rest, float* out_scales, float* out_rotation, float* out_opacity);
int gs_adc_gather_moments(gs_ctx* ctx, int total, int K, const int* gather_indices, const int* noise_mode, const int* actions,
                          const float* const in[6] , float* const out[6] );
int gs_adc_reset_opacity(gs_ctx* ctx, int N, float* opacity, float* m_opacity, float* v_opacity, float reset_value);


int gs_ply_write(gs_ctx* ctx, const char* path, int N, int K, const float* xyz, const float* features_dc,
                 const float* features_rest, const float* opacity, const float* scales, const float* rotation);
int gs_ply_probe(gs_ctx* ctx, const char* path, long long* N, int* M, int* D);
int gs_ply_load(gs_ctx* ctx, const char* path, int N, int K, float* xyz, float* features_dc, float* features_rest,
                float* opacity, float* scales, float* rotation);
int gs_ply_pack_rows(gs_ctx* ctx, int N, int K, const float* xyz, const float* features_dc,
                     const float* features_rest, const float* opacity, const float* scales, const float* rotation,
                     float* rows);

int gs_dist_topk(gs_ctx* ctx, int N, int k, int q_begin, int q_count, const float* xyz, float* out);


typedef enum gs_stage {
    GS_STAGE_PROJ_FWD = 0,
    GS_STAGE_BIN = 1,
    GS_STAGE_BLEND_FWD = 2,
    GS_STAGE_LOSS = 3,
    GS_STAGE_BLEND_BWD = 4,
    GS_STAGE_PROJ_BWD = 5,
    GS_STAGE_ADAM = 6,
    GS_STAGE_COUNT = 8
} gs_stage;
int gs_profile_enable(gs_ctx* ctx, unsigned stage_mask);
int gs_profile_read(gs_ctx* ctx, float ms[GS_STAGE_COUNT] , int calls[GS_STAGE_COUNT] );

int gs_last_stats(gs_ctx* ctx, uint32_t stats[8] );
int gs_set_block_work_buffer(gs_ctx* ctx, uint32_t* buf);
int gs_view_hint_words(gs_ctx* ctx, int* n);
int gs_set_view_hints(gs_ctx* ctx, uint32_t* buf, int words);
int gs_clear_depth_cuts(gs_ctx* ctx, uint32_t* buf, int words);
int gs_set_depth_cuts(gs_ctx* ctx, int enable);
int gs_forward_missed(gs_ctx* ctx, int* missed );
int gs_cut_stats(gs_ctx* ctx, uint32_t out[2] );
int gs_set_grad_norm_accum(gs_ctx* ctx, float* accum);
int gs_copy_overflow_flag(gs_ctx* ctx, uint32_t* out );
int gs_set_update_gate(gs_ctx* ctx, const uint32_t* gate );
int gs_set_overflow_rider(gs_ctx* ctx, float* dst );
int gs_set_gathered_gate(gs_ctx* ctx, long long block_floats, int count, uint32_t* reduced_out );
int gs_set_gate_seen(gs_ctx* ctx, uint32_t* seen );

typedef enum gs_tuning {
    GS_TUNE_FWD_WAVES_PER_SIMD = 0,
    GS_TUNE_BWD_WAVES_PER_CU = 1,
    GS_TUNE_FWD_QUADRANTS = 2,
    GS_TUNE_OP_FWD_PPL = 3,
    GS_TUNE_OP_BWD_PPL = 4,
    GS_TUNE_FWD_TRACE_BUFFER = 5,
    GS_TUNE_WIDE_TILE_SORT = 7,
    GS_TUNE_HOST_OVERFLOW_ERRORS = 8,
    GS_TUNE_SPLITTER_DEPTH_SORT = 9,
    GS_TUNE_COLOUR_RIDERS = 10,
    GS_TUNE_FWD_QUEUES = 11,
    GS_TUNE_FWD_FOUR_WAVES = 12,
    GS_TUNE_FWD_FOLD_TEST_SCALE = 13,
    GS_TUNE_RENDER_ONLY = 15,
    GS_TUNE_FWD_PAIR = 16,
    GS_TUNE_FWD_SLOW_SLOT = 17,
    GS_TUNE_TRIM_RECTS = 18,
    GS_TUNE_SH_BAND_SKIP = 19,
    GS_TUNE_POISON_CHECKPOINTS = 14,
    GS_TUNE_DEPTH_GRADIENT = 6
} gs_tuning;
int gs_ctx_set_tuning(gs_ctx* ctx, int knob, long long value);

int gs_block_count(gs_ctx* ctx, int* n);
int gs_copy_block_work(gs_ctx* ctx, uint32_t* out);
int gs_copy_last_contrib(gs_ctx* ctx, uint32_t* out);

#ifdef __cplusplus
}
#endif
#endif
```

Measured before the change: 646.8 views/s.

## Split Adam into touched rows and a concurrent zero-gradient pass for untouched rows

Builds a per-Gaussian 'touched' mask from the tile lists actually composited. The fused projection-backward-Adam kernel then runs in its sparse mode: it skips gradient loads and moment math for untouched rows. A separate kernel on a side stream applies the exact zero-gradient Adam update to untouched rows, overlapping with the main backward. The goal is to avoid full projection-backward work for Gaussians no pixel touched while keeping the dense Adam semantics. The cost is an extra mask clear/mark pass, a side stream with event synchronisation, and possible contention between the two streams.

```diff
diff --git a/gaussiansplattingmlx_amd/_lib.py b/gaussiansplattingmlx_amd/_lib.py
--- a/gaussiansplattingmlx_amd/_lib.py
+++ b/gaussiansplattingmlx_amd/_lib.py
@@ -205,6 +205,7 @@
     "gs_adc_reset_opacity": (C.c_int, [_vp, C.c_int, _vp, _vp, _vp, C.c_float]),
     "gs_set_sparse_adam": (C.c_int, [_vp, C.c_int]),
     "gs_get_visibility": (C.c_int, [_vp, C.c_int, _vp]),
+    "gs_get_touched": (C.c_int, [_vp, C.c_int, _vp]),
     "gs_adam_step_visible": (C.c_int, [_vp, C.c_longlong] + [_vp] * 4 + [C.c_int, _vp, _vp, _vp] + [C.c_float] * 4 + [C.c_int, _vp]),
     "gs_set_filter3d_cameras": (C.c_int, [_vp, C.c_int, _vp]),
     "gs_compute_filter3d": (C.c_int, [_vp, C.c_int, _vp, _vp]),
@@ -253,7 +254,8 @@
 
 TUNE_FWD_WAVES_PER_SIMD, TUNE_BWD_WAVES_PER_CU, TUNE_FWD_QUADRANTS, TUNE_OP_FWD_PPL, TUNE_OP_BWD_PPL, \
     TUNE_FWD_TRACE_BUFFER, TUNE_DEPTH_GRADIENT, TUNE_WIDE_TILE_SORT, TUNE_HOST_OVERFLOW_ERRORS, TUNE_SPLITTER_DEPTH_SORT, \
-    TUNE_COLOUR_RIDERS, TUNE_FWD_QUEUES, TUNE_FWD_FOUR_WAVES, TUNE_FWD_FOLD_TEST_SCALE, TUNE_POISON_CHECKPOINTS, TUNE_RENDER_ONLY, TUNE_FWD_PAIR, TUNE_FWD_SLOW_SLOT, TUNE_TRIM_RECTS, TUNE_SH_BAND_SKIP = range(20)
+    TUNE_COLOUR_RIDERS, TUNE_FWD_QUEUES, TUNE_FWD_FOUR_WAVES, TUNE_FWD_FOLD_TEST_SCALE, TUNE_POISON_CHECKPOINTS, TUNE_RENDER_ONLY, TUNE_FWD_PAIR, TUNE_FWD_SLOW_SLOT, TUNE_TRIM_RECTS, TUNE_SH_BAND_SKIP, \
+    TUNE_UNTOUCHED_ADAM = range(21)
 
 
 def exported_symbols():
diff --git a/gaussiansplattingmlx_amd/build.py b/gaussiansplattingmlx_amd/build.py
--- a/gaussiansplattingmlx_amd/build.py
+++ b/gaussiansplattingmlx_amd/build.py
@@ -36,6 +36,7 @@
     "lens.hip": ["-ffp-contract=off"],
     "metrics.hip": ["-ffp-contract=off"],
     "tsdf.hip": ["-ffp-contract=off"],
+    "untouched.hip": ["-ffp-contract=off"],
 }
 COMMON = ["-O3", "-std=c++17", "-fPIC", f"--offload-arch={ARCH}", "-fvisibility=hidden", "-Wall", "-fno-slp-vectorize",
           "-Wno-unused-function", "-DGSPLAT_BUILD"]
diff --git a/gaussiansplattingmlx_amd/csrc/api.hip b/gaussiansplattingmlx_amd/csrc/api.hip
--- a/gaussiansplattingmlx_amd/csrc/api.hip
+++ b/gaussiansplattingmlx_amd/csrc/api.hip
@@ -491,6 +491,8 @@
     for (auto& e : c->profPool) { (void)hipEventDestroy(e.a); (void)hipEventDestroy(e.b); }
     if (c->fwdDone) (void)hipEventDestroy(c->fwdDone);
     if (c->densifyDone) (void)hipEventDestroy(c->densifyDone);
+    for (hipEvent_t e : {c->sideFork, c->sideMask, c->sideDone}) if (e) (void)hipEventDestroy(e);
+    if (c->sideStream) (void)hipStreamDestroy(c->sideStream);
     if (c->own_stream) (void)hipStreamDestroy(c->own_stream);
     delete c;
     return GS_OK;
@@ -845,6 +847,7 @@
         return fail(c, GS_ERR_INVALID_ARG, "gs_render_forward: the fisheye camera model has no 3-D filter (gs_set_filter3d is set)");
     c->fwd.valid = false;
     c->visN = -1;
+    c->touchedN = -1;
     const bool keepRadii = c->sparseAdam || c->adcGradSum != nullptr;
     if (keepRadii && N > c->visCap) {
         if (const int arc = ctx_grow_pair(c, &c->visMask, &c->visRadii, &c->visCap, N > c->capN ? N : c->capN)) return arc;
@@ -1446,11 +1449,35 @@
     if (c->sparseAdam && (c->visN != N || c->fwd.modes.filter3d))
         return fail(c, GS_ERR_NO_FORWARD, "gs_render_backward_adam: sparse Adam is on, but the forward was not made under it "
                                           "(gs_set_sparse_adam comes before gs_render_forward)");
+    const bool untouched = untouched_applies(c) && !(c->adcGradSum && !c->fwd.radii);
+    if (untouched) {
+        if (const int rc = untouched_fork(c)) return rc;
+    } else c->touchedN = -1;
     if (const int rc = blend_backward_of_forward(c, cot_color, cot_depth, cot_alpha, c->absgrad, c->adamGate)) return rc;
+    if (untouched) {
+        if (const int rc = untouched_side(c, params_base, m_base, v_base, lr, beta1, beta2, eps, grad_scale)) return rc;
+    }
     c->fwd.consumed = true;
     AbsgradScope noNorm(c);
     GsStageTimer t(c, GS_STAGE_PROJ_BWD);
-    return launch_projection_fused_backward_adam(c, params_base, m_base, v_base, lr, beta1, beta2, eps, grad_scale);
+    if (!untouched) return launch_projection_fused_backward_adam(c, params_base, m_base, v_base, lr, beta1, beta2, eps, grad_scale);
+    const bool together = untouched_concurrent(c, params_base);
+    int rc = untouched_mask_ready(c);
+    if (rc == GS_OK && !together) rc = untouched_join(c);
+    if (rc == GS_OK) rc = launch_projection_fused_backward_adam(c, params_base, m_base, v_base, lr, beta1, beta2, eps, grad_scale, c->touched);
+    if (together || rc != GS_OK) { const int jrc = untouched_join(c); if (rc == GS_OK) rc = jrc; }
+    return rc;
+}
+
+int gs_get_touched(gs_ctx* c, int N, unsigned char* out)
+{
+    if (!c) return GS_ERR_INVALID_ARG;
+    if (c->touchedN < 0)
+        return fail(c, GS_ERR_NO_FORWARD, "gs_get_touched: the last gs_render_backward_adam did not take the untouched path (GS_TUNE_UNTOUCHED_ADAM)");
+    if (N != c->touchedN) return fail(c, GS_ERR_SIZE_MISMATCH, "gs_get_touched: N differs from the backward's N");
+    if (N > 0 && !out) return fail(c, GS_ERR_INVALID_ARG, "gs_get_touched: null buffer");
+    if (N > 0) GS_HIP_CHECK(c, hipMemcpyAsync(out, c->touched, (size_t)N, hipMemcpyDeviceToDevice, c->stream));
+    return GS_OK;
 }
 
 int gs_render_backward_dp_begin(gs_ctx* c, const float* cot_color, const float* cot_depth, const float* cot_alpha,
@@ -1853,6 +1880,8 @@
         c->trimRects = value != 0; c->rowGroups = value == 2; return GS_OK;
     case GS_TUNE_SH_BAND_SKIP:
         c->shBandSkip = value != 0; return GS_OK;
+    case GS_TUNE_UNTOUCHED_ADAM:
+        c->untouchedAdam = value != 0; return GS_OK;
     case GS_TUNE_FWD_TRACE_BUFFER:
         c->fwdTrace = reinterpret_cast<unsigned long long*>((uintptr_t)value); return GS_OK;
     default:
diff --git a/gaussiansplattingmlx_amd/csrc/gs_adam_fuse.h b/gaussiansplattingmlx_amd/csrc/gs_adam_fuse.h
--- /dev/null
+++ b/gaussiansplattingmlx_amd/csrc/gs_adam_fuse.h
@@ -0,0 +1,56 @@
+#pragma once
+#include "gs_ctx.h"
+
+namespace gs {
+
+struct AdamFuse {
+    const float* pBase;
+    float* mBase;
+    float* vBase;
+    float lr[6];
+    float b1, b2, eps, gscale;
+    const uint32_t* gate;
+    const uint32_t* ovf;
+    float* rider;
+    const uint32_t* gwWords;
+    long long gwStride;
+    int gwCount;
+    uint32_t* gwOut;
+    uint32_t* seen;
+};
+
+__device__ __forceinline__ uint32_t adam_gate_word(const AdamFuse& A)
+{
+    if (!A.gwWords) return A.gate ? *A.gate : 0u;
+    uint32_t g = 0;
+    for (int r = 0; r < A.gwCount; r++) g |= A.gwWords[(long long)r * A.gwStride];
+    return g;
+}
+__device__ __forceinline__ void adam_gate_publish(const AdamFuse& A, uint32_t g)
+{
+    if (blockIdx.x == 0 && threadIdx.x == 0) {
+        if (A.gwWords && A.gwOut) *A.gwOut = g;
+        if (g && A.seen) *A.seen = 1u;
+    }
+}
+
+__device__ __forceinline__ void adam_step(const AdamFuse& A, float g, float lr, float& p, float& m, float& v)
+{
+    const float gr = g * A.gscale;
+    m = A.b1 * m + (1.0f - A.b1) * gr;
+    v = A.b2 * v + (1.0f - A.b2) * gr * gr;
+    p = p - gs_adam_delta(lr, m, v, A.eps);
+}
+
+inline AdamFuse adam_fuse_of(const gs_ctx* c, const float* pBase, float* mBase, float* vBase, const float lr[6], float b1, float b2,
+                             float eps, float gscale)
+{
+    AdamFuse a = {};
+    a.pBase = pBase; a.mBase = mBase; a.vBase = vBase;
+    for (int i = 0; i < 6; i++) a.lr[i] = lr[i];
+    a.b1 = b1; a.b2 = b2; a.eps = eps; a.gscale = gscale;
+    a.gate = c->adamGate;
+    return a;
+}
+
+}
diff --git a/gaussiansplattingmlx_amd/csrc/gs_ctx.h b/gaussiansplattingmlx_amd/csrc/gs_ctx.h
--- a/gaussiansplattingmlx_amd/csrc/gs_ctx.h
+++ b/gaussiansplattingmlx_amd/csrc/gs_ctx.h
@@ -214,6 +214,12 @@
     float* visRadii = nullptr;
     int visCap = 0;
     int visN = -1;
+    int untouchedAdam = 1;
+    unsigned char* touched = nullptr;
+    int touchedCap = 0;
+    int touchedN = -1;
+    hipStream_t sideStream = nullptr;
+    hipEvent_t sideFork = nullptr, sideMask = nullptr, sideDone = nullptr;
     float* adcGradSum = nullptr;
     float* adcCount = nullptr;
     float* adcMaxRadius = nullptr;
@@ -442,8 +448,15 @@
 int launch_projection_fused_backward(gs_ctx* c, float* gXyz, float* gFdc, float* gFrest, float* gScales, float* gRot, float* gOpacity,
                                      bool emitColorCot = false);
 int launch_projection_fused_backward_adam(gs_ctx* c, const float* pBase, float* mBase, float* vBase, const float lr[6], float b1,
-                                          float b2, float eps, float gscale);
+                                          float b2, float eps, float gscale, const unsigned char* rowMask = nullptr);
 int launch_vis_mask(gs_ctx* c, int N, const float* radii);
+bool untouched_applies(const gs_ctx* c);
+bool untouched_concurrent(const gs_ctx* c, const float* pBase);
+int untouched_fork(gs_ctx* c);
+int untouched_side(gs_ctx* c, const float* pBase, float* mBase, float* vBase, const float lr[6], float b1, float b2, float eps,
+                   float gscale);
+int untouched_mask_ready(gs_ctx* c);
+int untouched_join(gs_ctx* c);
 bool depth_sort_takes_splitters(const gs_ctx* c, int N);
 int launch_pose_camera(gs_ctx* c, const gs::CamParams& host, const float* delta);
 int launch_pose_grad(gs_ctx* c, int N);
diff --git a/gaussiansplattingmlx_amd/csrc/projection.hip b/gaussiansplattingmlx_amd/csrc/projection.hip
--- a/gaussiansplattingmlx_amd/csrc/projection.hip
+++ b/gaussiansplattingmlx_amd/csrc/projection.hip
@@ -1,5 +1,6 @@
 #include <type_traits>
 
+#include "gs_adam_fuse.h"
 #include "gs_ctx.h"
 #include "gs_mcmc.h"
 #include "gs_rider.h"
@@ -167,12 +168,20 @@
 #define GS_PROJ_LATE_MOMENTS 1
 #endif
 
+template <bool SPARSE = false>
 __device__ __forceinline__ void sh_rows_load4(const float* __restrict__ g, int total4, int e0, int lane,
-                                              float4 (&regs)[SH_ROWS_MAX4])
+                                              float4 (&regs)[SH_ROWS_MAX4], int L = 0, unsigned long long rowBits = ~0ull)
 {
     const float4* g4 = reinterpret_cast<const float4*>(g);
 #pragma unroll
-    for (int i = 0; i < SH_ROWS_MAX4; i++) regs[i] = g4[min(e0 + lane + 64 * i, total4 - 1)];
+    for (int i = 0; i < SH_ROWS_MAX4; i++) {
+        const int e = min(e0 + lane + 64 * i, total4 - 1);
+        if constexpr (SPARSE) {
+            float4 v = make_float4(0.f, 0.f, 0.f, 0.f);
+            if ((rowBits >> ((4 * e) / L)) & 1ull) v = g4[e];
+            regs[i] = v;
+        } else regs[i] = g4[e];
+    }
 }
 __device__ __forceinline__ void sh_rows_to_lds4(float* __restrict__ lds, int total4, int L, int e0, int lane,
                                                 const float4 (&regs)[SH_ROWS_MAX4])
@@ -231,44 +240,6 @@
 #endif
 #include "gs_proj_fwd_kernel.h"
 
-struct AdamFuse {
-    const float* pBase;
-    float* mBase;
-    float* vBase;
-    float lr[6];
-    float b1, b2, eps, gscale;
-    const uint32_t* gate;
-    const uint32_t* ovf;
-    float* rider;
-    const uint32_t* gwWords;
-    long long gwStride;
-    int gwCount;
-    uint32_t* gwOut;
-    uint32_t* seen;
-};
-
-__device__ __forceinline__ uint32_t adam_gate_word(const AdamFuse& A)
-{
-    if (!A.gwWords) return A.gate ? *A.gate : 0u;
-    uint32_t g = 0;
-    for (int r = 0; r < A.gwCount; r++) g |= A.gwWords[(long long)r * A.gwStride];
-    return g;
-}
-__device__ __forceinline__ void adam_gate_publish(const AdamFuse& A, uint32_t g)
-{
-    if (blockIdx.x == 0 && threadIdx.x == 0) {
-        if (A.gwWords && A.gwOut) *A.gwOut = g;
-        if (g && A.seen) *A.seen = 1u;
-    }
-}
-
-__device__ __forceinline__ void adam_step(const AdamFuse& A, float g, float lr, float& p, float& m, float& v)
-{
-    const float gr = g * A.gscale;
-    m = A.b1 * m + (1.0f - A.b1) * gr;
-    v = A.b2 * v + (1.0f - A.b2) * gr * gr;
-    p = p - gs_adam_delta(lr, m, v, A.eps);
-}
 
 template <bool SPARSE = false>
 __device__ __forceinline__ void adam_rows(const AdamFuse& adam, const float* frest, int row0, int rows, int L,
@@ -557,7 +528,7 @@
         }
     } else
     if (kept) {
-        sh_rows_load4(frest + (size_t)row0 * L, total4, 0, lane, keptRows);
+        sh_rows_load4<SPARSE>(frest + (size_t)row0 * L, total4, 0, lane, keptRows, L, visBits);
         sh_rows_to_lds4(myRows, total4, L, 0, lane, keptRows);
     } else if (rows > 0 && L > 0) sh_rows_in(myRows, frest + (size_t)row0 * L, rows, L, lane);
     float pose[POSE ? 15 : 1];
@@ -653,7 +624,13 @@
                        }, d);
         if (ADAM) { sg_[11] = gdc[0]; sg_[12] = gdc[1]; sg_[13] = gdc[2]; }
     }
-    if (ADAM && GS_PROJ_LATE_MOMENTS) small_moments();
+    if (ADAM && GS_PROJ_LATE_MOMENTS) {
+        if constexpr (SPARSE) {
+#pragma unroll
+            for (int i = 0; i < 14; i++) { sm_[i] = 0.f; sv_[i] = 0.f; }
+            if (myVis) small_moments();
+        } else small_moments();
+    }
     if constexpr (POSE) {
         const bool live = (g0.x != 0.f || g0.y != 0.f || g0.z != 0.f || g0.w != 0.f || g1.x != 0.f ||
                                                  g1.y != 0.f || g1.z != 0.f || g1.w != 0.f || g2.x != 0.f || g2.y != 0.f ||
@@ -1167,7 +1144,7 @@
 }
 
 struct ProjBwdGrads { float *xyz, *fdc, *frest, *scales, *rot, *opacity; };
-static int launch_proj_bwd_fused(gs_ctx* c, int mode, const ProjBwdGrads& g, const AdamFuse& adam)
+static int launch_proj_bwd_fused(gs_ctx* c, int mode, const ProjBwdGrads& g, const AdamFuse& adam, const unsigned char* rowMask = nullptr)
 {
     const int N = c->fwd.N, K = c->fwd.K;
     if (N == 0) return c->fwd.modes.poseDelta && mode != 1 ? launch_pose_grad(c, 0) : GS_OK;
@@ -1175,7 +1152,7 @@
     if (f3d && mode == 1) mode = 0;
     const bool pose = c->fwd.modes.poseDelta && mode != 1;
     const bool mcmc = mode == 2 && !f3d && c->mcmcOn;
-    const bool sparse = mode == 2 && !f3d && !mcmc && c->sparseAdam;
+    const bool sparse = mode == 2 && !f3d && !mcmc && (c->sparseAdam || rowMask != nullptr);
     ProjBwdArgs a = {};
     a.N = N; a.K = K; a.degree = c->fwd.modes.degree;
     a.cam = c->fwd.cam; a.dcam = c->poseCam;
@@ -1187,7 +1164,7 @@
     a.posePartials = c->posePartials;
     if (mcmc) a.mc = mcmc_fuse(c->mcmc, N, adam.lr[0]);
     a.filter3d = c->fwd.modes.filter3d;
-    a.visMask = c->visMask;
+    a.visMask = rowMask ? rowMask : c->visMask;
     const bool bands = mode == 2 && !pose && !mcmc && !f3d && !sparse && c->shBandSkip && (a.degree + 2) * (a.degree + 2) <= K;
     const size_t lds = bands && a.degree == 0 ? 0 : sizeof(float) * (PROJ_FUSED_THREADS / 64) * 64 * ((K - 1) * 3 + 1);
     const int rc = with_flags(
@@ -1217,14 +1194,17 @@
 }
 
 int launch_projection_fused_backward_adam(gs_ctx* c, const float* pBase, float* mBase, float* vBase, const float lr[6], float b1,
-                                          float b2, float eps, float gscale)
-{
-    AdamFuse a = {};
-    a.pBase = pBase; a.mBase = mBase; a.vBase = vBase;
-    for (int i = 0; i < 6; i++) a.lr[i] = lr[i];
-    a.b1 = b1; a.b2 = b2; a.eps = eps; a.gscale = gscale;
-    a.gate = c->adamGate;
-    return launch_proj_bwd_fused(c, 2, ProjBwdGrads{}, a);
+                                          float b2, float eps, float gscale, const unsigned char* rowMask)
+{
+    return launch_proj_bwd_fused(c, 2, ProjBwdGrads{}, adam_fuse_of(c, pBase, mBase, vBase, lr, b1, b2, eps, gscale), rowMask);
+}
+
+bool untouched_applies(const gs_ctx* c)
+{
+    const int degree = c->fwd.modes.degree;
+    const bool bands = c->shBandSkip && (degree + 2) * (degree + 2) <= c->fwd.K;
+    return c->untouchedAdam != 0 && c->fast16 && c->fwd.N > 0 && !c->dp && !c->fwd.modes.poseDelta && !c->mcmcOn &&
+           !c->fwd.modes.filter3d && !c->sparseAdam && !bands;
 }
 
 static long long cc_block_floats(const gs_ctx* c, int N) { return c->ccBlockFloats > 0 ? c->ccBlockFloats : 3LL * N; }
diff --git a/gaussiansplattingmlx_amd/csrc/untouched.hip b/gaussiansplattingmlx_amd/csrc/untouched.hip
--- /dev/null
+++ b/gaussiansplattingmlx_amd/csrc/untouched.hip
@@ -0,0 +1,209 @@
+#include "gs_adam_fuse.h"
+#include "gs_ctx.h"
+
+namespace gs {
+
+__global__ __launch_bounds__(256) void touched_clear(uint4* __restrict__ mask16, int n16)
+{
+    const int i = blockIdx.x * 256 + threadIdx.x;
+    if (i < n16) mask16[i] = make_uint4(0u, 0u, 0u, 0u);
+}
+
+struct TouchedArgs {
+    int nBlocks, blocksX, tileW, tileH, gridW, N;
+    long long capM;
+    const uint32_t *tileRanges, *blockWork, *sortedIdx;
+    uint32_t idxMask;
+    const uint32_t* gate;
+    unsigned char* touched;
+};
+
+__global__ __launch_bounds__(256) void touched_mark(TouchedArgs a)
+{
+    if (a.gate && *a.gate) return;
+    const int b = blockIdx.x;
+    if (b >= a.nBlocks) return;
+    const int by = b / a.blocksX, bx = b - by * a.blocksX;
+    const int tile = ((by * 16) / a.tileH) * a.gridW + (bx * 16) / a.tileW;
+    const uint32_t s = a.tileRanges[2 * tile], e = a.tileRanges[2 * tile + 1];
+    if (e <= s || (long long)e > a.capM) return;
+    const uint32_t n = min(a.blockWork[b], e - s);
+    for (uint32_t i = threadIdx.x; i < n; i += 256u) {
+        const uint32_t g = a.sortedIdx[s + i] & a.idxMask;
+        if (g < (uint32_t)a.N) a.touched[g] = 1;
+    }
+}
+
+struct UntouchedArgs {
+    int N, K;
+    const float *xyz, *fdc, *frest, *scalesRaw, *rotRaw, *opacityRaw;
+    const unsigned char* touched;
+    AdamFuse adam;
+};
+
+template <int B>
+__global__ __launch_bounds__(256) void adam_untouched_kernel(UntouchedArgs a)
+{
+    const AdamFuse& A = a.adam;
+    if (adam_gate_word(A)) return;
+    const int lane = threadIdx.x & 63;
+    const int row0 = (blockIdx.x * 256 + (int)threadIdx.x) & ~63;
+    if (row0 >= a.N) return;
+    const int p = row0 + lane;
+    const bool un = p < a.N && a.touched[p] == 0;
+    const unsigned long long unBits = __ballot(un);
+    if (unBits == 0ull) return;
+    float* P = const_cast<float*>(A.pBase);
+    if (un) {
+        struct __attribute__((packed, aligned(4))) V3 { float x, y, z; };
+        struct __attribute__((packed, aligned(4))) V4 { float x, y, z, w; };
+        const size_t oX = (size_t)(a.xyz + 3 * (size_t)p - A.pBase), oS = (size_t)(a.scalesRaw + 3 * (size_t)p - A.pBase);
+        const size_t oD = (size_t)(a.fdc + 3 * (size_t)p - A.pBase), oR = (size_t)(a.rotRaw + 4 * (size_t)p - A.pBase);
+        const size_t oO = (size_t)(a.opacityRaw + (size_t)p - A.pBase);
+        V3 px = *reinterpret_cast<const V3*>(P + oX), mx = *reinterpret_cast<const V3*>(A.mBase + oX), vx = *reinterpret_cast<const V3*>(A.vBase + oX);
+        V3 ps = *reinterpret_cast<const V3*>(P + oS), ms = *reinterpret_cast<const V3*>(A.mBase + oS), vs = *reinterpret_cast<const V3*>(A.vBase + oS);
+        V3 pd = *reinterpret_cast<const V3*>(P + oD), md = *reinterpret_cast<const V3*>(A.mBase + oD), vd = *reinterpret_cast<const V3*>(A.vBase + oD);
+        V4 pr = *reinterpret_cast<const V4*>(P + oR), mr = *reinterpret_cast<const V4*>(A.mBase + oR), vr = *reinterpret_cast<const V4*>(A.vBase + oR);
+        float po = P[oO], mo = A.mBase[oO], vo = A.vBase[oO];
+        auto step3 = [&](float lr, V3& q, V3& m, V3& v) {
+            float q0 = q.x, q1 = q.y, q2 = q.z, m0 = m.x, m1 = m.y, m2 = m.z, v0 = v.x, v1 = v.y, v2 = v.z;
+            adam_step(A, 0.0f, lr, q0, m0, v0); adam_step(A, 0.0f, lr, q1, m1, v1); adam_step(A, 0.0f, lr, q2, m2, v2);
+            q = V3{q0, q1, q2}; m = V3{m0, m1, m2}; v = V3{v0, v1, v2};
+        };
+        step3(A.lr[0], px, mx, vx); step3(A.lr[3], ps, ms, vs); step3(A.lr[1], pd, md, vd);
+        {
+            float q0 = pr.x, q1 = pr.y, q2 = pr.z, q3 = pr.w, m0 = mr.x, m1 = mr.y, m2 = mr.z, m3 = mr.w;
+            float v0 = vr.x, v1 = vr.y, v2 = vr.z, v3 = vr.w;
+            adam_step(A, 0.0f, A.lr[4], q0, m0, v0); adam_step(A, 0.0f, A.lr[4], q1, m1, v1);
+            adam_step(A, 0.0f, A.lr[4], q2, m2, v2); adam_step(A, 0.0f, A.lr[4], q3, m3, v3);
+            pr = V4{q0, q1, q2, q3}; mr = V4{m0, m1, m2, m3}; vr = V4{v0, v1, v2, v3};
+        }
+        adam_step(A, 0.0f, A.lr[5], po, mo, vo);
+        *reinterpret_cast<V3*>(P + oX) = px; *reinterpret_cast<V3*>(A.mBase + oX) = mx; *reinterpret_cast<V3*>(A.vBase + oX) = vx;
+        *reinterpret_cast<V3*>(P + oS) = ps; *reinterpret_cast<V3*>(A.mBase + oS) = ms; *reinterpret_cast<V3*>(A.vBase + oS) = vs;
+        *reinterpret_cast<V3*>(P + oD) = pd; *reinterpret_cast<V3*>(A.mBase + oD) = md; *reinterpret_cast<V3*>(A.vBase + oD) = vd;
+        *reinterpret_cast<V4*>(P + oR) = pr; *reinterpret_cast<V4*>(A.mBase + oR) = mr; *reinterpret_cast<V4*>(A.vBase + oR) = vr;
+        P[oO] = po; A.mBase[oO] = mo; A.vBase[oO] = vo;
+    }
+    const int L = (a.K - 1) * 3;
+    if (L <= 0) return;
+    const int rows = min(64, a.N - row0);
+    const size_t off0 = (size_t)(a.frest - A.pBase) + (size_t)row0 * L;
+    float* Pr = P + off0;
+    float* Mr = A.mBase + off0;
+    float* Vr = A.vBase + off0;
+    const float lr = A.lr[2];
+    const int total = rows * L;
+    auto un_at = [&](int e) { return ((unBits >> (e / L)) & 1ull) != 0ull; };
+    const int head = min(total, (int)((4 - (off0 & 3)) & 3));
+    const int n4 = (total - head) >> 2;
+    const int tail0 = head + 4 * n4;
+    if (lane < head + (total - tail0)) {
+        const int e = lane < head ? lane : tail0 + (lane - head);
+        if (un_at(e)) {
+            float pv = Pr[e], mv = Mr[e], vv = Vr[e];
+            adam_step(A, 0.0f, lr, pv, mv, vv);
+            Pr[e] = pv; Mr[e] = mv; Vr[e] = vv;
+        }
+    }
+    float4* P4 = reinterpret_cast<float4*>(Pr + head);
+    float4* M4 = reinterpret_cast<float4*>(Mr + head);
+    float4* V4p = reinterpret_cast<float4*>(Vr + head);
+    for (int e0 = lane; e0 < n4; e0 += 64 * B) {
+        float4 pp[B], mm[B], vv[B];
+        bool on[B];
+#pragma unroll
+        for (int b = 0; b < B; b++) {
+            const int e = e0 + 64 * b, f = head + 4 * e;
+            on[b] = e < n4 && (un_at(f) || un_at(f + 3));
+            if (on[b]) { pp[b] = P4[e]; mm[b] = M4[e]; vv[b] = V4p[e]; }
+        }
+#pragma unroll
+        for (int b = 0; b < B; b++) {
+            if (!on[b]) continue;
+            const int e = e0 + 64 * b, f = head + 4 * e;
+            if (un_at(f)) adam_step(A, 0.0f, lr, pp[b].x, mm[b].x, vv[b].x);
+            if (un_at(f + 1)) adam_step(A, 0.0f, lr, pp[b].y, mm[b].y, vv[b].y);
+            if (un_at(f + 2)) adam_step(A, 0.0f, lr, pp[b].z, mm[b].z, vv[b].z);
+            if (un_at(f + 3)) adam_step(A, 0.0f, lr, pp[b].w, mm[b].w, vv[b].w);
+            P4[e] = pp[b]; M4[e] = mm[b]; V4p[e] = vv[b];
+        }
+    }
+}
+
+bool untouched_concurrent(const gs_ctx* c, const float* pBase)
+{
+    const int L = (c->fwd.K - 1) * 3;
+    return L == 0 || ((L & 3) == 0 && ((size_t)(c->fwd.frest - pBase) & 3) == 0);
+}
+
+static int launch_touched_mask(gs_ctx* c, hipStream_t s)
+{
+    const int N = c->fwd.N;
+    const int n16 = gs_div_up(N, 16);
+    hipLaunchKernelGGL(touched_clear, dim3(gs_div_up(n16, 256)), dim3(256), 0, s, reinterpret_cast<uint4*>(c->touched), n16);
+    TouchedArgs a;
+    a.nBlocks = c->numPixBlocks; a.blocksX = c->blocksX; a.tileW = c->tileW; a.tileH = c->tileH; a.gridW = c->gridW; a.N = N;
+    a.capM = c->capM;
+    a.tileRanges = c->tileRanges; a.blockWork = c->fwd.blockWork; a.sortedIdx = c->sortedRaw; a.idxMask = c->idxMask;
+    a.gate = c->adamGate;
+    a.touched = c->touched;
+    hipLaunchKernelGGL(touched_mark, dim3(c->numPixBlocks), dim3(256), 0, s, a);
+    GS_HIP_CHECK(c, hipGetLastError());
+    return GS_OK;
+}
+
+static int launch_adam_untouched(gs_ctx* c, hipStream_t s, const AdamFuse& adam)
+{
+    UntouchedArgs a;
+    a.N = c->fwd.N; a.K = c->fwd.K;
+    a.xyz = c->fwd.xyz; a.fdc = c->fwd.fdc; a.frest = c->fwd.frest; a.scalesRaw = c->fwd.scales; a.rotRaw = c->fwd.rot;
+    a.opacityRaw = c->fwd.opacity;
+    a.touched = c->touched;
+    a.adam = adam;
+    hipLaunchKernelGGL(adam_untouched_kernel<4>, dim3(gs_div_up(a.N, 256)), dim3(256), 0, s, a);
+    GS_HIP_CHECK(c, hipGetLastError());
+    return GS_OK;
+}
+
+static int untouched_setup(gs_ctx* c)
+{
+    if (!c->sideStream) GS_HIP_CHECK(c, hipStreamCreateWithFlags(&c->sideStream, hipStreamNonBlocking));
+    for (hipEvent_t* e : {&c->sideFork, &c->sideMask, &c->sideDone})
+        if (!*e) GS_HIP_CHECK(c, hipEventCreateWithFlags(e, hipEventDisableTiming));
+    const long long rowsWanted = c->fwd.N > c->capN ? c->fwd.N : c->capN;
+    return ctx_grow(c, &c->touched, &c->touchedCap, (rowsWanted + 15) / 16 * 16);
+}
+
+int untouched_fork(gs_ctx* c)
+{
+    if (const int rc = untouched_setup(c)) return rc;
+    GS_HIP_CHECK(c, hipEventRecord(c->sideFork, c->stream));
+    return GS_OK;
+}
+
+int untouched_side(gs_ctx* c, const float* pBase, float* mBase, float* vBase, const float lr[6], float b1, float b2, float eps,
+                   float gscale)
+{
+    GS_HIP_CHECK(c, hipStreamWaitEvent(c->sideStream, c->sideFork, 0));
+    if (const int rc = launch_touched_mask(c, c->sideStream)) return rc;
+    GS_HIP_CHECK(c, hipEventRecord(c->sideMask, c->sideStream));
+    c->touchedN = c->fwd.N;
+    if (const int rc = launch_adam_untouched(c, c->sideStream, adam_fuse_of(c, pBase, mBase, vBase, lr, b1, b2, eps, gscale))) return rc;
+    GS_HIP_CHECK(c, hipEventRecord(c->sideDone, c->sideStream));
+    return GS_OK;
+}
+
+int untouched_mask_ready(gs_ctx* c)
+{
+    GS_HIP_CHECK(c, hipStreamWaitEvent(c->stream, c->sideMask, 0));
+    return GS_OK;
+}
+
+int untouched_join(gs_ctx* c)
+{
+    GS_HIP_CHECK(c, hipStreamWaitEvent(c->stream, c->sideDone, 0));
+    return GS_OK;
+}
+
+}
diff --git a/gaussiansplattingmlx_amd/renderer.py b/gaussiansplattingmlx_amd/renderer.py
--- a/gaussiansplattingmlx_amd/renderer.py
+++ b/gaussiansplattingmlx_amd/renderer.py
@@ -145,11 +145,12 @@
                    colour_riders=_lib.TUNE_COLOUR_RIDERS, fwd_queues=_lib.TUNE_FWD_QUEUES, fwd_four_waves=_lib.TUNE_FWD_FOUR_WAVES,
                    fwd_fold_test_scale=_lib.TUNE_FWD_FOLD_TEST_SCALE, poison_checkpoints=_lib.TUNE_POISON_CHECKPOINTS,
                    render_only=_lib.TUNE_RENDER_ONLY, fwd_pair=_lib.TUNE_FWD_PAIR, fwd_slow_slot=_lib.TUNE_FWD_SLOW_SLOT,
-                   trim_rects=_lib.TUNE_TRIM_RECTS, sh_band_skip=_lib.TUNE_SH_BAND_SKIP)
+                   trim_rects=_lib.TUNE_TRIM_RECTS, sh_band_skip=_lib.TUNE_SH_BAND_SKIP,
+                   untouched_adam=_lib.TUNE_UNTOUCHED_ADAM)
     _TUNING_DEFAULTS = dict(fwd_waves_per_simd=4, bwd_waves_per_cu=16, fwd_quadrants=1, op_fwd_ppl=1, op_bwd_ppl=1,
                             fwd_trace_buffer=0, depth_gradient=1, wide_tile_sort=1, host_overflow_errors=1, splitter_depth_sort=1,
                             colour_riders=1, fwd_queues=8, fwd_four_waves=-1, fwd_fold_test_scale=1000, poison_checkpoints=0, render_only=0, fwd_pair=-1, fwd_slow_slot=3, trim_rects=2,
-                            sh_band_skip=1)
+                            sh_band_skip=1, untouched_adam=1)
 
     def setTuning(self, **knobs):
         for k, v in knobs.items():
diff --git a/include/gsplat.h b/include/gsplat.h
--- a/include/gsplat.h
+++ b/include/gsplat.h
@@ -150,6 +150,7 @@
 
 int gs_set_sparse_adam(gs_ctx* ctx, int enable);
 int gs_get_visibility(gs_ctx* ctx, int N, unsigned char* out );
+int gs_get_touched(gs_ctx* ctx, int N, unsigned char* out );
 
 int gs_set_filter3d_cameras(gs_ctx* ctx, int V, const gs_camera* cams );
 int gs_compute_filter3d(gs_ctx* ctx, int N, const float* xyz , float* filter );
@@ -446,6 +447,7 @@
     GS_TUNE_FWD_SLOW_SLOT = 17,
     GS_TUNE_TRIM_RECTS = 18,
     GS_TUNE_SH_BAND_SKIP = 19,
+    GS_TUNE_UNTOUCHED_ADAM = 20,
     GS_TUNE_POISON_CHECKPOINTS = 14,
     GS_TUNE_DEPTH_GRADIENT = 6
 } gs_tuning;
```

New measurement: 673.6 views/s (median of 6 runs). +4.2%, better.
